# IST-DASLab/torch_cgx

Hardware: AMD Instinct MI355X
Metric: DDP samples/sec ResNet-50 4-bit (higher is better)
Workload: dtype bf16; 1 GPU; model=resnet50, global_batch=256, input=3x224x224, parallelism=dp1, backend=cgx, bits=4, bucket_size=1024, compression_active=False

## Files before the change

### csrc/bindings.cc

```cpp
#include <torch/extension.h>

#include <ATen/hip/impl/HIPStreamMasqueradingAsCUDA.h>
#include <torch/csrc/utils/pybind.h>

#include <ATen/hip/impl/HIPGuardImplMasqueradingAsCUDA.h>

#include <cstring>
#include <functional>
#include <thread>
#include <tuple>

#include "backend.h"
#include "bn_plan.h"
#include "collectives.h"
#include "reducer.h"

namespace cgx {
namespace {

void run_rank_threads(int ws, int dev,
                      const std::function<void(int, hipStream_t)>& body,
                      const std::function<void()>& abort) {
  std::vector<hipStream_t> qs(ws, nullptr);
  for (auto& s : qs)
    CGX_HIP_CHECK(hipStreamCreateWithFlags(&s, hipStreamNonBlocking));
  std::vector<std::exception_ptr> errs(ws);
  {
    py::gil_scoped_release nogil;
    std::vector<std::thread> th;
    for (int r = 0; r < ws; r++) {
      th.emplace_back([&, r] {
        try {
          c10::hip::HIPGuardMasqueradingAsCUDA g(dev);
          body(r, qs[r]);
        } catch (...) {
          errs[r] = std::current_exception();
          abort();
        }
      });
    }
    for (auto& t : th) t.join();
  }
  (void)hipDeviceSynchronize();
  for (auto s : qs)
    if (s) (void)hipStreamDestroy(s);
  for (int r = 0; r < ws; r++)
    if (errs[r]) std::rethrow_exception(errs[r]);
}

struct LoopbackWorld {
  std::vector<std::unique_ptr<LoopbackHub>> hubs;
  std::vector<std::unique_ptr<LoopbackTransport>> trs;
  std::vector<Reducer> ranks;

  LoopbackWorld(int ws, int local_size) {
    ranks.resize(ws);
    LoopbackHub* world = hub(ws);
    for (int r = 0; r < ws; r++) ranks[r].flat.emplace(r, ws, tr(world, r));
    if (local_size == 0) return;
    const int nodes = ws / local_size;
    LoopbackHub* cross = hub(nodes);
    for (int nd = 0; nd < nodes; nd++) {
      LoopbackHub* intra = hub(local_size);
      for (int lr = 0; lr < local_size; lr++) {
        Reducer& red = ranks[nd * local_size + lr];
        red.intra.emplace(lr, local_size, tr(intra, lr));
        red.leader = lr == 0;
        if (red.leader)
          red.cross.emplace(nd, nodes, tr(cross, nd), true);
      }
    }
  }
  void abort() {
    for (auto& h : hubs) h->abort();
  }

 private:
  LoopbackHub* hub(int world) {
    hubs.push_back(std::make_unique<LoopbackHub>(world));
    return hubs.back().get();
  }
  Transport* tr(LoopbackHub* h, int rank) {
    trs.push_back(std::make_unique<LoopbackTransport>(h, rank));
    return trs.back().get();
  }
};

void run_loopback(
    const std::vector<at::Tensor>& tensors, int local_size,
    const std::function<hipStream_t(Reducer&, hipStream_t, int)>& body) {
  const int ws = (int)tensors.size();
  TORCH_CHECK(ws >= 2, "loopback: need >= 2 per-rank tensors");
  TORCH_CHECK(local_size == 0 || (ws % local_size == 0 && ws / local_size >= 2),
              "loopback: hierarchical world must be n_nodes*local_size with "
              ">= 2 nodes");
  for (const auto& t : tensors) {
    TORCH_CHECK(t.is_cuda() && t.is_contiguous(),
                "loopback: CUDA contiguous tensors required");
    TORCH_CHECK(t.device() == tensors[0].device() &&
                    t.numel() == tensors[0].numel() &&
                    t.scalar_type() == tensors[0].scalar_type(),
                "loopback: tensors must match in device/numel/dtype");
  }
  const int dev = tensors[0].device().index();
  c10::hip::HIPGuardMasqueradingAsCUDA guard(dev);
  LoopbackWorld world(ws, local_size);
  run_rank_threads(
      ws, dev,
      [&](int r, hipStream_t qs) {
        hipStream_t fin = body(world.ranks[r], qs, r);
        CGX_HIP_CHECK(hipStreamSynchronize(fin));
        CGX_HIP_CHECK(hipStreamSynchronize(qs));
        world.ranks[r].for_each_stream(
            [](hipStream_t s) { CGX_HIP_CHECK(hipStreamSynchronize(s)); });
      },
      [&] { world.abort(); });
}

struct Resolved {
  explicit Resolved(int64_t numel)
      : matched(Registry::get().next(numel, nullptr, &info)) {}
  Registry::BucketInfo info;
  bool matched;
};

void py_loopback_allreduce(std::vector<at::Tensor> buckets) {
  const Resolved reg(buckets.empty() ? 0 : buckets[0].numel());
  run_loopback(buckets, 0,
               [&](Reducer& red, hipStream_t qs, int r) {
                 return red.allreduce(buckets[r], qs, &reg.info, reg.matched);
               });
}

void py_loopback_allreduce_multi(
    std::vector<std::vector<at::Tensor>> steps) {
  TORCH_CHECK(!steps.empty(), "loopback_allreduce_multi: no steps");
  const int ws = (int)steps[0].size();
  const int64_t numel = steps[0][0].numel();
  for (auto& st : steps) {
    TORCH_CHECK((int)st.size() == ws && st[0].numel() == numel,
                "loopback_allreduce_multi: ragged steps");
  }
  const Resolved reg(numel);
  run_loopback(steps[0], 0,
               [&](Reducer& red, hipStream_t qs, int r) {
                 hipStream_t fin = qs;
                 for (auto& st : steps)
                   fin = red.allreduce(st[r], qs, &reg.info, reg.matched);
                 return fin;
               });
}

void py_loopback_broadcast(std::vector<at::Tensor> tensors, int64_t root) {
  run_loopback(tensors, 0,
               [&](Reducer& red, hipStream_t qs, int r) {
                 return red.flat->engine->broadcast(tensors[r], (int)root,
                                                    red.flat->tr, qs);
               });
}

void py_loopback_hierarchical(std::vector<at::Tensor> buckets,
                              int64_t local_size) {
  TORCH_CHECK(local_size >= 1, "loopback_hierarchical: local_size >= 1");
  const Resolved reg(buckets.empty() ? 0 : buckets[0].numel());
  run_loopback(buckets, (int)local_size,
               [&](Reducer& red, hipStream_t qs, int r) {
                 return red.allreduce(buckets[r], qs, &reg.info, reg.matched);
               });
}

void py_loopback_collective(
    const std::string& name, std::vector<std::vector<at::Tensor>> inputs,
    std::vector<std::vector<at::Tensor>> outputs, int64_t root,
    std::vector<std::vector<int64_t>> in_splits,
    std::vector<std::vector<int64_t>> out_splits) {
  const int ws = (int)inputs.size();
  TORCH_CHECK(ws >= 1 && (int)outputs.size() == ws && root >= 0 && root < ws,
              "loopback_collective: one input and one output list per rank "
              "and a root among them");
  TORCH_CHECK((in_splits.empty() || (int)in_splits.size() == ws) &&
                  (out_splits.empty() || (int)out_splits.size() == ws),
              "loopback_collective: splits are per rank, or empty");
  in_splits.resize(ws);
  out_splits.resize(ws);
  std::function<size_t(int)> n_in, n_out;
  std::function<void(Transport*, int, hipStream_t)> call;
  const auto one = [](int) { return (size_t)1; };
  const auto all = [ws](int) { return (size_t)ws; };
  const auto at_root = [ws, root](int r) { return r == root ? (size_t)ws : 0; };
  if (name == "allgather") {
    n_in = one; n_out = all;
    call = [&](Transport* tr, int r, hipStream_t s) {
      coll::allgather(tr, r, ws, inputs[r][0], outputs[r], s);
    };
  } else if (name == "gather") {
    n_in = one; n_out = at_root;
    call = [&](Transport* tr, int r, hipStream_t s) {
      coll::gather(tr, r, ws, (int)root, inputs[r][0], outputs[r], s);
    };
  } else if (name == "scatter") {
    n_in = at_root; n_out = one;
    call = [&](Transport* tr, int r, hipStream_t s) {
      coll::scatter(tr, r, ws, (int)root, inputs[r], outputs[r][0], s);
    };
  } else if (name == "alltoall") {
    n_in = all; n_out = all;
    call = [&](Transport* tr, int r, hipStream_t s) {
      coll::alltoall(tr, r, ws, inputs[r], outputs[r], s);
    };
  } else if (name == "alltoall_base") {
    n_in = one; n_out = one;
    call = [&](Transport* tr, int r, hipStream_t s) {
      coll::alltoall_base(tr, r, ws, inputs[r][0], outputs[r][0], in_splits[r],
                          out_splits[r], s);
    };
  } else {
    TORCH_CHECK(false, "loopback_collective: unknown collective '", name, "'");
  }
  c10::optional<at::Device> device;
  for (int r = 0; r < ws; r++) {
    TORCH_CHECK(inputs[r].size() == n_in(r) && outputs[r].size() == n_out(r),
                "loopback_collective: rank ", r, " of ", name, " takes ",
                n_in(r), " input and ", n_out(r), " output tensors");
    for (const auto* ts : {&inputs[r], &outputs[r]})
      for (const at::Tensor& t : *ts) {
        TORCH_CHECK(t.is_cuda() && t.is_contiguous(),
                    "loopback_collective: CUDA contiguous tensors required");
        if (!device) device = t.device();
        TORCH_CHECK(t.device() == *device,
                    "loopback_collective: tensors must share one device");
      }
  }
  const int dev = device->index();
  c10::hip::HIPGuardMasqueradingAsCUDA guard(dev);
  CGX_HIP_CHECK(hipStreamSynchronize(
      c10::hip::getCurrentHIPStreamMasqueradingAsCUDA(dev).stream()));
  LoopbackHub hub(ws);
  std::vector<LoopbackTransport> trs;
  for (int r = 0; r < ws; r++) trs.emplace_back(&hub, r);
  run_rank_threads(
      ws, dev,
      [&](int r, hipStream_t s) {
        call(&trs[r], r, s);
        CGX_HIP_CHECK(hipStreamSynchronize(s));
      },
      [&] { hub.abort(); });
}

template <typename Desc>
at::Tensor upload(const std::vector<Desc>& descs,
                  const std::vector<int64_t>& cum, at::Device device) {
  const size_t desc_bytes = sizeof(Desc) * descs.size();
  const size_t cum_bytes = sizeof(int64_t) * cum.size();
  std::vector<char> host(desc_bytes + cum_bytes);
  std::memcpy(host.data(), descs.data(), desc_bytes);
  std::memcpy(host.data() + desc_bytes, cum.data(), cum_bytes);
  return at::from_blob(host.data(), {(int64_t)host.size()},
                       at::TensorOptions().dtype(at::kByte))
      .to(device);
}

void dequantize_slice(const at::Tensor& comp, at::Tensor& out, int64_t bits,
                      int64_t bucket_size, bool skip_incomplete,
                      int64_t src_stride, int nsrc, bool add) {
  const DType dt = dtype_of(out);
  auto stream =
      c10::hip::getCurrentHIPStreamMasqueradingAsCUDA(out.device().index());
  const std::vector<DequantSlice> slices{
      DequantSlice{comp.data_ptr<uint8_t>(), out.data_ptr(), out.numel(),
                   (int)bits, (int)bucket_size, skip_incomplete}};
  for (const DequantGroup& g :
       route_dequantize(slices, dt, src_stride, nsrc, add)) {
    auto dev = upload(g.descs, {}, out.device());
    launch(g, static_cast<const DequantDesc*>(dev.data_ptr()), dt,
           stream.stream());
  }
}

at::Tensor py_quantize(at::Tensor x, int64_t bits, int64_t bucket_size,
                       bool stochastic, int64_t seed, bool skip_incomplete,
                       c10::optional<at::Tensor> feedback) {
  TORCH_CHECK(x.is_cuda() && x.is_contiguous(), "quantize: CUDA contiguous");
  TORCH_CHECK(bits >= 1 && bits <= 8, "quantize: bits in [1,8]");
  TORCH_CHECK(bucket_size >= 1, "quantize: bucket_size >= 1");
  void* fbp = nullptr;
  if (feedback.has_value()) {
    TORCH_CHECK(feedback->is_cuda() && feedback->is_contiguous() &&
                    feedback->numel() == x.numel() &&
                    feedback->scalar_type() == x.scalar_type(),
                "quantize: feedback must match x");
    TORCH_CHECK(bucket_size % 8 == 0,
                "quantize: error feedback requires bucket_size % 8 == 0");
    fbp = feedback->data_ptr();
  }
  const DType dt = dtype_of(x);
  const int64_t n = x.numel();
  const int64_t bytes =
      buffer_size(n, dt, (int)bits, (int)bucket_size, skip_incomplete);
  auto out = at::zeros({std::max<int64_t>(bytes, 1)},
                       at::TensorOptions().dtype(at::kByte).device(x.device()));
  auto stream =
      c10::hip::getCurrentHIPStreamMasqueradingAsCUDA(x.device().index());
  for (const QuantGroup& g : route_quantize({QuantSlice{
           x.data_ptr(), out.data_ptr<uint8_t>(), fbp, n, (int)bits,
           (int)bucket_size, skip_incomplete}})) {
    auto dev = upload(g.descs, g.cum, x.device());
    const char* devp = static_cast<const char*>(dev.data_ptr());
    launch(g, reinterpret_cast<const QuantDesc*>(devp),
           reinterpret_cast<const int64_t*>(devp +
                                            sizeof(QuantDesc) * g.descs.size()),
           dt, (uint64_t)seed, stochastic, stream.stream());
  }
  return out;
}

void py_dequantize(at::Tensor comp, at::Tensor out, int64_t bits,
                   int64_t bucket_size, bool add, bool skip_incomplete) {
  TORCH_CHECK(comp.is_cuda() && out.is_cuda() && out.is_contiguous());
  dequantize_slice(comp, out, bits, bucket_size, skip_incomplete,
                   0, 1, add);
}

void py_dequantize_multi(at::Tensor comp, at::Tensor out, int64_t bits,
                         int64_t bucket_size, bool add) {
  TORCH_CHECK(comp.is_cuda() && comp.dim() == 2 && comp.is_contiguous());
  TORCH_CHECK(out.is_cuda() && out.is_contiguous());
  dequantize_slice(comp, out, bits, bucket_size, false,
                   comp.stride(0), (int)comp.size(0), add);
}

int64_t py_buffer_size(int64_t n, at::ScalarType st, int64_t bits,
                       int64_t bucket_size, bool skip_incomplete) {
  return buffer_size(n, dtype_of(st), (int)bits, (int)bucket_size,
                     skip_incomplete);
}

py::list py_route_quantize(
    const std::vector<std::tuple<uint64_t, uint64_t, uint64_t, int64_t, int,
                                 int, bool>>& slices) {
  std::vector<QuantSlice> qs;
  for (const auto& [in, out, fb, n, bits, bucket, skip] : slices)
    qs.push_back(QuantSlice{reinterpret_cast<const void*>(in),
                            reinterpret_cast<uint8_t*>(out),
                            reinterpret_cast<void*>(fb), n, bits, bucket,
                            skip});
  py::list groups;
  for (const QuantGroup& g : route_quantize(qs)) {
    py::list descs;
    for (const QuantDesc& d : g.descs)
      descs.append(py::make_tuple(reinterpret_cast<uint64_t>(d.in),
                                  reinterpret_cast<uint64_t>(d.out),
                                  reinterpret_cast<uint64_t>(d.fb), d.n,
                                  d.bucket, d.flags));
    groups.append(py::make_tuple(g.bits, g.kind, descs, g.cum, g.any_residual,
                                 g.max_gpl));
  }
  return groups;
}

py::list py_route_dequantize(
    const std::vector<std::tuple<uint64_t, uint64_t, int64_t, int, int,
                                 bool>>& slices,
    at::ScalarType st, int64_t src_stride, int nsrc, bool add) {
  std::vector<DequantSlice> ds;
  for (const auto& [in, out, n, bits, bucket, skip] : slices)
    ds.push_back(DequantSlice{reinterpret_cast<const uint8_t*>(in),
                              reinterpret_cast<void*>(out), n, bits, bucket,
                              skip});
  py::list groups;
  for (const DequantGroup& g :
       route_dequantize(ds, dtype_of(st), src_stride, nsrc, add)) {
    py::list descs;
    for (const DequantDesc& d : g.descs)
      descs.append(py::make_tuple(reinterpret_cast<uint64_t>(d.in),
                                  reinterpret_cast<uint64_t>(d.out), d.n,
                                  d.src_stride, d.bucket, d.nsrc, d.add,
                                  d.flags));
    groups.append(py::make_tuple(g.bits, g.kind, descs, g.total_groups,
                                 g.any_residual));
  }
  return groups;
}

std::pair<std::vector<int64_t>, std::vector<int64_t>> py_partition(
    int64_t num_elements, int64_t world_size,
    std::vector<int64_t> layer_numels, int64_t esize) {
  std::vector<int64_t> offs, szs;
  partition(num_elements, (int)world_size, layer_numels, (int)esize, &offs,
            &szs);
  return {offs, szs};
}

using PyView = std::tuple<uint64_t, int64_t, int, int>;
std::vector<LayerView> to_views(const std::vector<PyView>& views) {
  std::vector<LayerView> out;
  for (const auto& [off, numel, bits, bucket] : views)
    out.push_back(LayerView{reinterpret_cast<char*>(off), numel, bits, bucket});
  return out;
}

py::tuple py_plan_bucket(const std::vector<int64_t>& layer_numels,
                         const std::vector<std::pair<int, int>>& layer_cfgs,
                         at::ScalarType st, int64_t fusion_bytes,
                         int64_t min_elems, double fake_ratio, bool dummy) {
  TORCH_CHECK(layer_numels.size() == layer_cfgs.size(),
              "plan_bucket: one (bits, bucket_size) per layer");
  const int es = elem_size(dtype_of(st));
  EngineConfig cfg;
  cfg.fusion_bytes = fusion_bytes;
  cfg.min_elems = min_elems;
  cfg.fake_ratio = fake_ratio;
  cfg.dummy = dummy;
  std::vector<LayerView> views;
  int64_t off = 0;
  for (size_t i = 0; i < layer_numels.size(); i++) {
    views.push_back(LayerView{reinterpret_cast<char*>(off * es),
                              layer_numels[i], layer_cfgs[i].first,
                              layer_cfgs[i].second});
    off += layer_numels[i];
  }
  const BucketPlan bp = plan_bucket(views, cfg, es);
  py::list uncomp, chunks;
  for (const auto& [ptr, cnt] : bp.uncomp)
    uncomp.append(py::make_tuple(reinterpret_cast<uint64_t>(ptr), cnt));
  for (const auto& chunk : bp.chunks) {
    py::list vs;
    for (const LayerView& v : chunk)
      vs.append(py::make_tuple(reinterpret_cast<uint64_t>(v.data), v.numel,
                               v.bits, v.bucket_size));
    chunks.append(vs);
  }
  return py::make_tuple(uncomp, chunks);
}

py::tuple py_plan_chunk(const std::vector<PyView>& views, at::ScalarType st,
                        int ws, bool skip_incomplete) {
  TORCH_CHECK(ws >= 1, "plan_chunk: ws >= 1");
  const ChunkPlan pl =
      plan_chunk(to_views(views), dtype_of(st), ws, skip_incomplete);
  py::list rs;
  for (const auto& slices : pl.rs) {
    py::list r;
    for (const Slice& s : slices)
      r.append(py::make_tuple(reinterpret_cast<uint64_t>(s.data), s.n, s.bits,
                              s.bucket, s.comp_off, s.skip_incomplete,
                              s.fb_off));
    rs.append(r);
  }
  return py::make_tuple(pl.offs, pl.szs, pl.comp, rs);
}


bool bn_tensor_ok(const at::Tensor& t) {
  return t.is_cuda() && t.scalar_type() == at::kBFloat16 && t.dim() == 4 &&
         t.numel() > 0 && t.is_contiguous(at::MemoryFormat::ChannelsLast) &&
         reinterpret_cast<uintptr_t>(t.data_ptr()) % 16 == 0;
}

BnPlan bn_plan_of(const at::Tensor& t) {
  return bn_plan(t.numel() / t.size(1), t.size(1));
}

bool py_bn_eligible(const at::Tensor& x) {
  return bn_tensor_ok(x) && bn_plan_of(x).eligible;
}

float* bn_channel_vec(const at::Tensor& t, int64_t c, const char* what) {
  TORCH_CHECK(t.is_cuda() && t.scalar_type() == at::kFloat &&
                  t.is_contiguous() && t.numel() == c,
              "bn_act: ", what, " must be a contiguous fp32 CUDA vector of ",
              c, " elements");
  return t.data_ptr<float>();
}

at::Tensor bn_workspace(const BnPlan& p, const at::Tensor& like) {
  return at::empty({2 * p.partial_floats + p.grid},
                   like.options().dtype(at::kFloat));
}

std::tuple<at::Tensor, at::Tensor, at::Tensor, c10::optional<at::Tensor>>
py_bn_act_forward(const at::Tensor& x, const c10::optional<at::Tensor>& identity,
                  const at::Tensor& weight, const at::Tensor& bias,
                  at::Tensor running_mean, at::Tensor running_var,
                  double momentum, double eps, bool relu) {
  TORCH_CHECK(py_bn_eligible(x), "bn_act_forward: input is not eligible");
  const BnPlan p = bn_plan_of(x);
  const int64_t c = p.channels;
  if (identity.has_value())
    TORCH_CHECK(bn_tensor_ok(*identity) && identity->sizes() == x.sizes() &&
                    identity->device() == x.device(),
                "bn_act_forward: identity must match the input");
  c10::hip::HIPGuardMasqueradingAsCUDA guard(x.device().index());
  auto out = at::empty(x.sizes(), x.options(), at::MemoryFormat::ChannelsLast);
  auto stats = x.options().dtype(at::kFloat);
  auto mean = at::empty({c}, stats), invstd = at::empty({c}, stats);
  c10::optional<at::Tensor> mask;
  if (relu) mask = at::empty({x.numel() / 8}, x.options().dtype(at::kByte));
  auto part = bn_workspace(p, x);
  BnForwardArgs a;
  a.x = x.data_ptr();
  a.identity = identity.has_value() ? identity->data_ptr() : nullptr;
  a.weight = bn_channel_vec(weight, c, "weight");
  a.bias = bn_channel_vec(bias, c, "bias");
  a.running_mean = bn_channel_vec(running_mean, c, "running_mean");
  a.running_var = bn_channel_vec(running_var, c, "running_var");
  a.momentum = (float)momentum;
  a.eps = (float)eps;
  a.relu = relu;
  a.out = out.data_ptr();
  a.mean = mean.data_ptr<float>();
  a.invstd = invstd.data_ptr<float>();
  a.mask = relu ? mask->data_ptr<uint8_t>() : nullptr;
  a.part = part.data_ptr<float>();
  launch_bn_forward(
      p, a, c10::hip::getCurrentHIPStreamMasqueradingAsCUDA(
                x.device().index()).stream());
  return {out, mean, invstd, mask};
}

std::tuple<at::Tensor, at::Tensor, at::Tensor, c10::optional<at::Tensor>>
py_bn_act_backward(at::Tensor dy, const at::Tensor& x, const at::Tensor& mean,
                   const at::Tensor& invstd, const at::Tensor& weight,
                   const c10::optional<at::Tensor>& mask, bool has_identity) {
  TORCH_CHECK(py_bn_eligible(x), "bn_act_backward: input is not eligible");
  const BnPlan p = bn_plan_of(x);
  const int64_t c = p.channels;
  TORCH_CHECK(dy.is_cuda() && dy.device() == x.device() &&
                  dy.scalar_type() == at::kBFloat16 && dy.sizes() == x.sizes(),
              "bn_act_backward: dy must match the input");
  c10::hip::HIPGuardMasqueradingAsCUDA guard(x.device().index());
  if (!bn_tensor_ok(dy)) dy = dy.contiguous(at::MemoryFormat::ChannelsLast);
  if (!bn_tensor_ok(dy)) dy = dy.clone(at::MemoryFormat::ChannelsLast);
  if (mask.has_value())
    TORCH_CHECK(mask->is_cuda() && mask->scalar_type() == at::kByte &&
                    mask->is_contiguous() && mask->numel() == x.numel() / 8,
                "bn_act_backward: mask must hold one bit per element");
  auto dx = at::empty(x.sizes(), x.options(), at::MemoryFormat::ChannelsLast);
  auto stats = x.options().dtype(at::kFloat);
  auto dgamma = at::empty({c}, stats), dbeta = at::empty({c}, stats);
  c10::optional<at::Tensor> didentity;
  if (has_identity)
    didentity = mask.has_value()
                    ? at::empty(x.sizes(), x.options(),
                                at::MemoryFormat::ChannelsLast)
                    : dy;
  auto part = bn_workspace(p, x);
  BnBackwardArgs a;
  a.dy = dy.data_ptr();
  a.x = x.data_ptr();
  a.mean = bn_channel_vec(mean, c, "mean");
  a.invstd = bn_channel_vec(invstd, c, "invstd");
  a.weight = bn_channel_vec(weight, c, "weight");
  a.mask = mask.has_value() ? mask->data_ptr<uint8_t>() : nullptr;
  a.dx = dx.data_ptr();
  a.didentity =
      has_identity && mask.has_value() ? didentity->data_ptr() : nullptr;
  a.dgamma = dgamma.data_ptr<float>();
  a.dbeta = dbeta.data_ptr<float>();
  a.part = part.data_ptr<float>();
  launch_bn_backward(
      p, a, c10::hip::getCurrentHIPStreamMasqueradingAsCUDA(
                x.device().index()).stream());
  return {dx, dgamma, dbeta, didentity};
}

hipStream_t bn_stream(const at::Tensor& x) {
  return c10::hip::getCurrentHIPStreamMasqueradingAsCUDA(x.device().index())
      .stream();
}

at::Tensor bn_dense_dy(at::Tensor dy) {
  if (!bn_tensor_ok(dy)) dy = dy.contiguous(at::MemoryFormat::ChannelsLast);
  if (!bn_tensor_ok(dy)) dy = dy.clone(at::MemoryFormat::ChannelsLast);
  return dy;
}

std::tuple<at::Tensor, at::Tensor, at::Tensor, at::Tensor, at::Tensor,
           c10::optional<at::Tensor>>
py_bn_act2_forward(const at::Tensor& x3, const at::Tensor& xd,
                   const at::Tensor& weight3, const at::Tensor& bias3,
                   at::Tensor running_mean3, at::Tensor running_var3,
                   double momentum3, double eps3, const at::Tensor& weightd,
                   const at::Tensor& biasd, at::Tensor running_meand,
                   at::Tensor running_vard, double momentumd, double epsd,
                   bool relu) {
  TORCH_CHECK(py_bn_eligible(x3), "bn_act2_forward: input is not eligible");
  TORCH_CHECK(bn_tensor_ok(xd) && xd.sizes() == x3.sizes() &&
                  xd.device() == x3.device(),
              "bn_act2_forward: both inputs must have the same shape");
  const BnPlan p = bn_plan_of(x3);
  const int64_t c = p.channels;
  c10::hip::HIPGuardMasqueradingAsCUDA guard(x3.device().index());
  auto out = at::empty(x3.sizes(), x3.options(), at::MemoryFormat::ChannelsLast);
  auto stats = x3.options().dtype(at::kFloat);
  auto mean3 = at::empty({c}, stats), invstd3 = at::empty({c}, stats);
  auto meand = at::empty({c}, stats), invstdd = at::empty({c}, stats);
  c10::optional<at::Tensor> mask;
  if (relu) mask = at::empty({x3.numel() / 8}, x3.options().dtype(at::kByte));
  auto part = at::empty({2 * (2 * p.partial_floats + p.grid)}, stats);
  BnJoinArgs j{};
  j.a.x = x3.data_ptr();
  j.a.weight = bn_channel_vec(weight3, c, "weight");
  j.a.bias = bn_channel_vec(bias3, c, "bias");
  j.a.running_mean = bn_channel_vec(running_mean3, c, "running_mean");
  j.a.running_var = bn_channel_vec(running_var3, c, "running_var");
  j.a.momentum = (float)momentum3;
  j.a.eps = (float)eps3;
  j.a.mean = mean3.data_ptr<float>();
  j.a.invstd = invstd3.data_ptr<float>();
  j.b.x = xd.data_ptr();
  j.b.weight = bn_channel_vec(weightd, c, "identity weight");
  j.b.bias = bn_channel_vec(biasd, c, "identity bias");
  j.b.running_mean = bn_channel_vec(running_meand, c, "identity running_mean");
  j.b.running_var = bn_channel_vec(running_vard, c, "identity running_var");
  j.b.momentum = (float)momentumd;
  j.b.eps = (float)epsd;
  j.b.mean = meand.data_ptr<float>();
  j.b.invstd = invstdd.data_ptr<float>();
  j.relu = relu;
  j.out = out.data_ptr();
  j.mask = relu ? mask->data_ptr<uint8_t>() : nullptr;
  j.part = part.data_ptr<float>();
  launch_bn_join_forward(p, j, bn_stream(x3));
  return {out, mean3, invstd3, meand, invstdd, mask};
}

std::tuple<at::Tensor, at::Tensor, at::Tensor, at::Tensor, at::Tensor,
           at::Tensor>
py_bn_act2_backward(at::Tensor dy, const at::Tensor& x3, const at::Tensor& xd,
                    const at::Tensor& mean3, const at::Tensor& invstd3,
                    const at::Tensor& weight3, const at::Tensor& meand,
                    const at::Tensor& invstdd, const at::Tensor& weightd,
                    const c10::optional<at::Tensor>& mask) {
  TORCH_CHECK(py_bn_eligible(x3), "bn_act2_backward: input is not eligible");
  TORCH_CHECK(bn_tensor_ok(xd) && xd.sizes() == x3.sizes() &&
                  xd.device() == x3.device(),
              "bn_act2_backward: both inputs must have the same shape");
  const BnPlan p = bn_plan_of(x3);
  const int64_t c = p.channels;
  TORCH_CHECK(dy.is_cuda() && dy.device() == x3.device() &&
                  dy.scalar_type() == at::kBFloat16 && dy.sizes() == x3.sizes(),
              "bn_act2_backward: dy must match the input");
  c10::hip::HIPGuardMasqueradingAsCUDA guard(x3.device().index());
  dy = bn_dense_dy(dy);
  if (mask.has_value())
    TORCH_CHECK(mask->is_cuda() && mask->scalar_type() == at::kByte &&
                    mask->is_contiguous() && mask->numel() == x3.numel() / 8,
                "bn_act2_backward: mask must hold one bit per element");
  auto dx3 = at::empty(x3.sizes(), x3.options(), at::MemoryFormat::ChannelsLast);
  auto dxd = at::empty(x3.sizes(), x3.options(), at::MemoryFormat::ChannelsLast);
  auto stats = x3.options().dtype(at::kFloat);
  auto dgamma3 = at::empty({c}, stats), dbeta3 = at::empty({c}, stats);
  auto dgammad = at::empty({c}, stats), dbetad = at::empty({c}, stats);
  auto part = at::empty({3 * p.partial_floats}, stats);
  BnJoinArgs j{};
  j.a.x = x3.data_ptr();
  j.a.mean = bn_channel_vec(mean3, c, "mean");
  j.a.invstd = bn_channel_vec(invstd3, c, "invstd");
  j.a.weight = bn_channel_vec(weight3, c, "weight");
  j.a.dx = dx3.data_ptr();
  j.a.dgamma = dgamma3.data_ptr<float>();
  j.a.dbeta = dbeta3.data_ptr<float>();
  j.b.x = xd.data_ptr();
  j.b.mean = bn_channel_vec(meand, c, "identity mean");
  j.b.invstd = bn_channel_vec(invstdd, c, "identity invstd");
  j.b.weight = bn_channel_vec(weightd, c, "identity weight");
  j.b.dx = dxd.data_ptr();
  j.b.dgamma = dgammad.data_ptr<float>();
  j.b.dbeta = dbetad.data_ptr<float>();
  j.dy = dy.data_ptr();
  j.mask = mask.has_value() ? mask->data_ptr<uint8_t>() : nullptr;
  j.part = part.data_ptr<float>();
  launch_bn_join_backward(p, j, bn_stream(x3));
  return {dx3, dxd, dgamma3, dbeta3, dgammad, dbetad};
}

BnPoolPlan bn_pool_plan_of(const at::Tensor& x) {
  return bn_pool_plan(x.size(0), x.size(2), x.size(3), x.size(1));
}

std::tuple<at::Tensor, at::Tensor, at::Tensor, at::Tensor>
py_bn_act_pool_forward(const at::Tensor& x, const at::Tensor& weight,
                       const at::Tensor& bias, at::Tensor running_mean,
                       at::Tensor running_var, double momentum, double eps) {
  TORCH_CHECK(py_bn_eligible(x), "bn_act_pool_forward: input is not eligible");
  const BnPlan p = bn_plan_of(x);
  const BnPoolPlan g = bn_pool_plan_of(x);
  const int64_t c = p.channels;
  c10::hip::HIPGuardMasqueradingAsCUDA guard(x.device().index());
  auto out = at::empty({x.size(0), c, g.oh, g.ow}, x.options(),
                       at::MemoryFormat::ChannelsLast);
  auto arg = at::empty({x.size(0), c, g.oh, g.ow},
                       x.options().dtype(at::kByte),
                       at::MemoryFormat::ChannelsLast);
  auto stats = x.options().dtype(at::kFloat);
  auto mean = at::empty({c}, stats), invstd = at::empty({c}, stats);
  auto part = bn_workspace(p, x);
  BnPoolArgs a{};
  a.x = x.data_ptr();
  a.weight = bn_channel_vec(weight, c, "weight");
  a.bias = bn_channel_vec(bias, c, "bias");
  a.running_mean = bn_channel_vec(running_mean, c, "running_mean");
  a.running_var = bn_channel_vec(running_var, c, "running_var");
  a.momentum = (float)momentum;
  a.eps = (float)eps;
  a.mean = mean.data_ptr<float>();
  a.invstd = invstd.data_ptr<float>();
  a.out = out.data_ptr();
  a.arg = arg.data_ptr<uint8_t>();
  a.part = part.data_ptr<float>();
  launch_bn_pool_forward(p, g, a, bn_stream(x));
  return {out, mean, invstd, arg};
}

std::tuple<at::Tensor, at::Tensor, at::Tensor>
py_bn_act_pool_backward(at::Tensor dy, const at::Tensor& x,
                        const at::Tensor& mean, const at::Tensor& invstd,
                        const at::Tensor& weight, const at::Tensor& arg) {
  TORCH_CHECK(py_bn_eligible(x), "bn_act_pool_backward: input is not eligible");
  const BnPlan p = bn_plan_of(x);
  const BnPoolPlan g = bn_pool_plan_of(x);
  const int64_t c = p.channels;
  const std::vector<int64_t> pooled = {x.size(0), c, g.oh, g.ow};
  TORCH_CHECK(dy.is_cuda() && dy.device() == x.device() &&
                  dy.scalar_type() == at::kBFloat16 && dy.sizes() == at::IntArrayRef(pooled),
              "bn_act_pool_backward: dy must have the pooled shape");
  TORCH_CHECK(arg.is_cuda() && arg.device() == x.device() &&
                  arg.scalar_type() == at::kByte && arg.sizes() == at::IntArrayRef(pooled) &&
                  arg.is_contiguous(at::MemoryFormat::ChannelsLast) &&
                  reinterpret_cast<uintptr_t>(arg.data_ptr()) % 8 == 0,
              "bn_act_pool_backward: arg must be the forward's");
  c10::hip::HIPGuardMasqueradingAsCUDA guard(x.device().index());
  dy = bn_dense_dy(dy);
  auto dx = at::empty(x.sizes(), x.options(), at::MemoryFormat::ChannelsLast);
  auto stats = x.options().dtype(at::kFloat);
  auto dgamma = at::empty({c}, stats), dbeta = at::empty({c}, stats);
  auto part = bn_workspace(p, x);
  BnPoolArgs a{};
  a.x = x.data_ptr();
  a.mean = bn_channel_vec(mean, c, "mean");
  a.invstd = bn_channel_vec(invstd, c, "invstd");
  a.weight = bn_channel_vec(weight, c, "weight");
  a.arg = arg.data_ptr<uint8_t>();
  a.dy = dy.data_ptr();
  a.dx = dx.data_ptr();
  a.dgamma = dgamma.data_ptr<float>();
  a.dbeta = dbeta.data_ptr<float>();
  a.part = part.data_ptr<float>();
  launch_bn_pool_backward(p, g, a, bn_stream(x));
  return {dx, dgamma, dbeta};
}

std::tuple<at::Tensor, at::Tensor> py_bn_pool_geometry(int64_t h, int64_t w) {
  TORCH_CHECK(h >= 1 && w >= 1 && h * w <= kBnMaxRows, "bn_pool_geometry: bad");
  const BnPoolPlan g = bn_pool_plan(1, h, w, 8);
  auto opt = at::TensorOptions().dtype(at::kLong);
  auto windows = at::full({(int64_t)g.oh * g.ow, 9}, -1, opt);
  auto covers = at::full({h * w, 4, 2}, -1, opt);
  int64_t* wi = windows.data_ptr<int64_t>();
  int64_t* co = covers.data_ptr<int64_t>();
  for (int oh = 0; oh < g.oh; oh++)
    for (int ow = 0; ow < g.ow; ow++)
      for (int k = 0; k < 9; k++) {
        const int ih = pool_in(oh, k / 3), iw = pool_in(ow, k % 3);
        if (ih >= 0 && ih < g.h && iw >= 0 && iw < g.w)
          wi[((int64_t)oh * g.ow + ow) * 9 + k] = (int64_t)ih * g.w + iw;
      }
  for (int ih = 0; ih < g.h; ih++)
    for (int iw = 0; iw < g.w; iw++) {
      int n = 0;
      for (int oh = pool_cover_lo(ih); oh <= pool_cover_hi(ih, g.oh); oh++)
        for (int ow = pool_cover_lo(iw); ow <= pool_cover_hi(iw, g.ow); ow++) {
          int64_t* e = co + (((int64_t)ih * g.w + iw) * 4 + n++) * 2;
          e[0] = (int64_t)oh * g.ow + ow;
          e[1] = pool_k(ih, oh) * 3 + pool_k(iw, ow);
        }
    }
  return {windows, covers};
}

py::dict py_bn_plan(int64_t rows, int64_t channels) {
  const BnPlan p = bn_plan(rows, channels);
  py::dict d;
  d["eligible"] = p.eligible;
  d["threads"] = kBnThreads;
  d["cgs"] = p.cgs;
  d["tile_cgs"] = p.tc;
  d["ctiles"] = p.ctiles;
  d["rows_per_iter"] = p.rln;
  d["splits"] = p.splits;
  d["grid"] = p.grid;
  d["rows_per_thread"] = p.rows_per_thread;
  d["partial_floats"] = p.partial_floats;
  return d;
}

at::Tensor py_bn_sweep_indices(int64_t rows, int64_t channels) {
  const BnPlan p = bn_plan(rows, channels);
  TORCH_CHECK(p.eligible, "bn_sweep_indices: shape is not eligible");
  auto out = at::full({(int64_t)p.grid * kBnThreads, p.rows_per_thread + 1},
                      -1, at::TensorOptions().dtype(at::kLong));
  int64_t* o = out.data_ptr<int64_t>();
  const int64_t width = p.rows_per_thread + 1;
  for (int wg = 0; wg < p.grid; wg++)
    for (int tid = 0; tid < kBnThreads; tid++) {
      const BnSweep sw = bn_sweep(p, wg, tid);
      int64_t k = 0;
      for (int64_t r = sw.row; r < p.rows; r += sw.stride, k++) {
        TORCH_CHECK(k < width, "bn_sweep_indices: run longer than planned");
        o[((int64_t)wg * kBnThreads + tid) * width + k] = bn_vec(p, r, sw.cg);
      }
    }
  return out;
}

std::vector<int64_t> py_bn_partial_offsets(int64_t rows, int64_t channels,
                                           int wg) {
  const BnPlan p = bn_plan(rows, channels);
  TORCH_CHECK(p.eligible && wg >= 0 && wg < p.grid, "bn_partial_offsets: bad");
  std::vector<int64_t> offs;
  for (int tid = 0; tid < p.tc; tid++) {
    const BnSweep sw = bn_sweep(p, wg, tid);
    const int64_t o = bn_partial_offset(p, wg, sw.cg);
    for (int j = 0; j < 8; j++) offs.push_back(o + j);
  }
  return offs;
}

void py_register_layer(int64_t bucket_idx, int64_t layer_idx, int64_t numel,
                       int64_t bits, int64_t bucket_size) {
  Registry::get().register_layer((int)bucket_idx, (int)layer_idx, numel,
                                 (int)bits, (int)bucket_size);
}

void py_set_bits(int64_t bucket_idx, int64_t layer_idx, int64_t bits) {
  Registry::get().set_bits((int)bucket_idx, (int)layer_idx, (int)bits);
}

void py_set_bucket(int64_t bucket_idx, int64_t layer_idx,
                   int64_t bucket_size) {
  Registry::get().set_bucket_size((int)bucket_idx, (int)layer_idx,
                                  (int)bucket_size);
}

}
}

PYBIND11_MODULE(TORCH_EXTENSION_NAME, m) {
  py::class_<cgx::ProcessGroupCGX,
             c10::intrusive_ptr<cgx::ProcessGroupCGX>, c10d::Backend>(
      m, "ProcessGroupCGX")
      .def(py::init<c10::intrusive_ptr<c10d::Store>, int, int,
                    c10::intrusive_ptr<c10d::Backend>>(),
           py::arg("store"), py::arg("rank"), py::arg("size"),
           py::arg("cpu_delegate") = nullptr);

  m.def("register_layer", &cgx::py_register_layer, py::arg("bucket_idx"),
        py::arg("layer_idx"), py::arg("layer_numel"), py::arg("bits"),
        py::arg("bucket_size"));
  m.def("set_quantization_bits", &cgx::py_set_bits);
  m.def("set_quantization_bucket_size", &cgx::py_set_bucket);
  m.def("clear_registry", [] { cgx::Registry::get().clear(); });
  m.def("registry_match",
        [](int64_t numel, int64_t key) {
          cgx::Registry::BucketInfo info;
          const bool ok = cgx::Registry::get().next(
              numel, reinterpret_cast<const void*>(key), &info);
          return py::make_tuple(ok, ok ? info.idx : -1);
        },
        py::arg("numel"), py::arg("key") = 0);
  m.def("registry_snapshot", [] {
    py::list out;
    auto& reg = cgx::Registry::get();
    for (const auto& b : reg.snapshot()) {
      py::list numels, cfgs;
      for (auto n : b.numels) numels.append(n);
      for (const auto& c : b.cfgs)
        cfgs.append(py::make_tuple(c.bits, c.bucket_size));
      out.append(py::make_tuple(b.idx, numels, cfgs));
    }
    return out;
  });

  m.def("parse_engine_config", [] {
    auto c = cgx::EngineConfig::from_env();
    py::dict d;
    d["fusion_bytes"] = c.fusion_bytes;
    d["min_elems"] = c.min_elems;
    d["default_bits"] = c.default_bits;
    d["default_bucket"] = c.default_bucket;
    d["stochastic"] = c.stochastic;
    d["inner_ring"] = c.ring;
    d["cross_ring"] = c.cross_ring;
    d["debug_a2a"] = c.debug_a2a;
    d["fake_ratio"] = c.fake_ratio;
    d["skip_incomplete"] = c.skip_incomplete;
    d["dummy"] = c.dummy;
    d["intra_compress"] = c.intra_compress;
    d["intra_broadcast"] = c.intra_broadcast;
    d["error_feedback"] = c.error_feedback;
    return d;
  });
  m.def("env_flag", &cgx::env_flag, py::arg("name"),
        py::arg("default") = false,
        "Test seam: the textual boolean parser (only \"0\" is false).");
  m.def("env_int", &cgx::env_int, py::arg("name"), py::arg("default"),
        "Test seam: the numeric parser behind the `!= 0` booleans.");
  m.def("loopback_allreduce", &cgx::py_loopback_allreduce, py::arg("buckets"),
        "Run Reducer::allreduce (flat) at world_size=len(buckets) on one GPU "
        "via the loopback transport; buckets[r] is rank r's flat bucket "
        "tensor, reduced in place.");
  m.def("loopback_broadcast", &cgx::py_loopback_broadcast, py::arg("tensors"),
        py::arg("root") = 0,
        "Run the production Engine::broadcast at world_size=len(tensors) on "
        "one GPU via the loopback transport.");
  m.def("loopback_allreduce_multi", &cgx::py_loopback_allreduce_multi,
        py::arg("steps"),
        "Multiple allreduce steps on persistent engines (steps[s][r] = rank "
        "r's bucket at step s, reduced in place); error-feedback residuals "
        "carry across steps.");
  m.def("loopback_hierarchical", &cgx::py_loopback_hierarchical,
        py::arg("buckets"), py::arg("local_size"),
        "Run Reducer::allreduce, the backend's per-bucket call, for "
        "n_nodes*local_size ranks on one GPU via loopback transports: intra "
        "allreduce -> leader cross reduction -> intra broadcast, or the "
        "flat path under CGX_INTRA_BROADCAST=0.");
  m.def("loopback_collective", &cgx::py_loopback_collective, py::arg("name"),
        py::arg("inputs"), py::arg("outputs"), py::arg("root") = 0,
        py::arg("in_splits") = std::vector<std::vector<int64_t>>{},
        py::arg("out_splits") = std::vector<std::vector<int64_t>>{},
        "Run one of the backend's p2p collectives (allgather, gather, "
        "scatter, alltoall, alltoall_base) at world_size=len(inputs) on one "
        "GPU via the loopback transport; inputs[r] / outputs[r] are rank r's "
        "tensor lists, in_splits[r] / out_splits[r] its alltoall_base splits.");
  m.def("quantize", &cgx::py_quantize, py::arg("x"), py::arg("bits"),
        py::arg("bucket_size"), py::arg("stochastic") = false,
        py::arg("seed") = 0, py::arg("skip_incomplete") = false,
        py::arg("feedback") = py::none());
  m.def("dequantize", &cgx::py_dequantize, py::arg("comp"), py::arg("out"),
        py::arg("bits"), py::arg("bucket_size"), py::arg("add") = false,
        py::arg("skip_incomplete") = false);
  m.def("dequantize_multi", &cgx::py_dequantize_multi, py::arg("comp"),
        py::arg("out"), py::arg("bits"), py::arg("bucket_size"),
        py::arg("add") = false);
  m.def("compute_topology",
        [](const c10::intrusive_ptr<c10d::Store>& store, int rank, int size,
           const std::string& hostname) {
          auto t = cgx::compute_topology(store, rank, size, hostname);
          return std::make_tuple(t.node_id, t.local_rank, t.local_size,
                                 t.n_nodes, t.uniform);
        },
        "Exchange hostnames through the store -> (node_id, local_rank, "
        "local_size, n_nodes, uniform)");
  m.def("buffer_size", &cgx::py_buffer_size, py::arg("n"), py::arg("dtype"),
        py::arg("bits"), py::arg("bucket_size"),
        py::arg("skip_incomplete") = false);
  m.def("partition", &cgx::py_partition);
  m.def("plan_bucket", &cgx::py_plan_bucket, py::arg("layer_numels"),
        py::arg("layer_cfgs"), py::arg("dtype"), py::arg("fusion_bytes"),
        py::arg("min_elems"), py::arg("fake_ratio") = 1.0,
        py::arg("dummy") = false,
        "Test seam: the bucket plan for layers laid out back to back from "
        "byte offset 0 -> (uncomp [(byte_off, count)], chunks [[(byte_off, "
        "numel, bits, bucket)]]).");
  m.def("plan_chunk", &cgx::py_plan_chunk, py::arg("views"), py::arg("dtype"),
        py::arg("ws"), py::arg("skip_incomplete") = false,
        "Test seam: the rank plan of one chunk [(byte_off, numel, bits, "
        "bucket)] -> (offs, szs, comp, rs [[(byte_off, n, bits, bucket, "
        "comp_off, skip_incomplete, fb_off)]]).");
  m.def("route_quantize", &cgx::py_route_quantize, py::arg("slices"),
        "Test seam: the launch router's quantize plan for "
        "[(in, out, fb, n, bits, bucket, skip_incomplete)] (pointers as "
        "ints) -> [(bits, kind, descs, cum, any_residual, max_gpl)].");
  m.def("route_dequantize", &cgx::py_route_dequantize, py::arg("slices"),
        py::arg("dtype"), py::arg("src_stride") = 0, py::arg("nsrc") = 1,
        py::arg("add") = false,
        "Test seam: the launch router's dequantize plan for "
        "[(in, out, n, bits, bucket, skip_incomplete)] -> "
        "[(bits, kind, descs, total_groups, any_residual)].");
  m.def("bn_act_forward", &cgx::py_bn_act_forward, py::arg("x"),
        py::arg("identity"), py::arg("weight"), py::arg("bias"),
        py::arg("running_mean"), py::arg("running_var"), py::arg("momentum"),
        py::arg("eps"), py::arg("relu"),
        "Training-mode BatchNorm2d of a channels_last bf16 tensor, fused with "
        "an optional residual add and ReLU -> (out, mean, invstd, mask | "
        "None); updates the running statistics in place.");
  m.def("bn_act_backward", &cgx::py_bn_act_backward, py::arg("dy"),
        py::arg("x"), py::arg("mean"), py::arg("invstd"), py::arg("weight"),
        py::arg("mask"), py::arg("has_identity"),
        "Backward of bn_act_forward -> (dx, dgamma, dbeta, didentity | None).");
  m.def("bn_act2_forward", &cgx::py_bn_act2_forward,
        "relu(bn3(x3) + bn_d(xd)) with both BatchNorms in training mode: "
        "(x3, xd, weight3, bias3, running_mean3, running_var3, momentum3, "
        "eps3, weightd, biasd, running_meand, running_vard, momentumd, epsd, "
        "relu) -> (out, mean3, invstd3, meand, invstdd, mask | None).");
  m.def("bn_act2_backward", &cgx::py_bn_act2_backward,
        "Backward of bn_act2_forward: (dy, x3, xd, mean3, invstd3, weight3, "
        "meand, invstdd, weightd, mask) -> (dx3, dxd, dgamma3, dbeta3, "
        "dgammad, dbetad).");
  m.def("bn_act_pool_forward", &cgx::py_bn_act_pool_forward, py::arg("x"),
        py::arg("weight"), py::arg("bias"), py::arg("running_mean"),
        py::arg("running_var"), py::arg("momentum"), py::arg("eps"),
        "max_pool2d(relu(bn(x)), 3, 2, 1) in training mode -> (pooled, mean, "
        "invstd, arg); arg is one byte per pooled element.");
  m.def("bn_act_pool_backward", &cgx::py_bn_act_pool_backward, py::arg("dy"),
        py::arg("x"), py::arg("mean"), py::arg("invstd"), py::arg("weight"),
        py::arg("arg"),
        "Backward of bn_act_pool_forward -> (dx, dgamma, dbeta).");
  m.def("bn_pool_geometry", &cgx::py_bn_pool_geometry, py::arg("h"),
        py::arg("w"),
        "Test seam: (windows [oh*ow, 9], covers [h*w, 4, 2]) of the stem's "
        "3x3/2/1 pooling as the kernels index it.");
  m.def("bn_eligible", &cgx::py_bn_eligible, py::arg("x"),
        "True where the fused BatchNorm kernels take `x`: CUDA, bf16, dense "
        "channels_last, and a shape bn_plan calls eligible.");
  m.def("bn_plan", &cgx::py_bn_plan, py::arg("rows"), py::arg("channels"),
        "Test seam: the launch geometry of the fused BatchNorm kernels for a "
        "[rows, channels] activation.");
  m.def("bn_sweep_indices", &cgx::py_bn_sweep_indices, py::arg("rows"),
        py::arg("channels"),
        "Test seam: [grid*threads, rows_per_thread+1] int64, the 16-byte "
        "vector indices every thread visits (-1: none).");
  m.def("bn_partial_offsets", &cgx::py_bn_partial_offsets, py::arg("rows"),
        py::arg("channels"), py::arg("wg"),
        "Test seam: the partial-buffer floats workgroup `wg` writes.");
  m.attr("FLAG_SKIP_INCOMPLETE") = cgx::kFlagSkipIncomplete;
  m.attr("FLAG_TAIL_ONLY") = cgx::kFlagTailOnly;
  m.attr("KIND_FAST") = (int)cgx::kFast;
  m.attr("KIND_GENERIC") = (int)cgx::kGeneric;
  m.attr("KIND_TWO_PASS") = (int)cgx::kTwoPass;
  m.attr("KIND_SUB") = (int)cgx::kSub;
}
```

### csrc/bn_kernels.hip

```cpp
#include <hip/hip_runtime.h>

#include "bn_plan.h"
#include "check.h"

namespace cgx {
namespace {

constexpr int kT = kBnThreads;

__device__ inline void unpack8(const uint4& v, float (&f)[8]) {
  f[0] = __uint_as_float(v.x << 16);
  f[1] = __uint_as_float(v.x & 0xffff0000u);
  f[2] = __uint_as_float(v.y << 16);
  f[3] = __uint_as_float(v.y & 0xffff0000u);
  f[4] = __uint_as_float(v.z << 16);
  f[5] = __uint_as_float(v.z & 0xffff0000u);
  f[6] = __uint_as_float(v.w << 16);
  f[7] = __uint_as_float(v.w & 0xffff0000u);
}

__device__ inline unsigned bf16_bits(float f) {
  const unsigned u = __float_as_uint(f);
  if ((u & 0x7fffffffu) > 0x7f800000u) return (u >> 16) | 0x40u;
  return (u + 0x7fffu + ((u >> 16) & 1u)) >> 16;
}

__device__ inline uint4 pack8(const unsigned (&b)[8]) {
  return make_uint4(b[0] | (b[1] << 16), b[2] | (b[3] << 16),
                    b[4] | (b[5] << 16), b[6] | (b[7] << 16));
}

__device__ inline unsigned half_of(const uint4& v, int j) {
  const unsigned w = j < 2 ? v.x : j < 4 ? v.y : j < 6 ? v.z : v.w;
  return (j & 1) ? w >> 16 : w & 0xffffu;
}

template <int K>
__device__ inline void load_k(float (&dst)[K], const float* src) {
#pragma unroll
  for (int j = 0; j < K; j++) dst[j] = src[j];
}


template <int K>
struct Moments {
  float n = 0.f;
  float mean[K] = {};
  float m2[K] = {};

  __device__ void push(const float (&x)[K]) {
    n += 1.f;
    const float inv = __builtin_amdgcn_rcpf(n);
#pragma unroll
    for (int j = 0; j < K; j++) {
      const float d = x[j] - mean[j];
      mean[j] = fmaf(d, inv, mean[j]);
      m2[j] = fmaf(d, x[j] - mean[j], m2[j]);
    }
  }

  __device__ void merge(float nb, const float (&mb)[K], const float (&m2b)[K]) {
    const float nt = n + nb;
    const float fb = nt > 0.f ? nb / nt : 0.f;
    const float w = n * fb;
#pragma unroll
    for (int j = 0; j < K; j++) {
      const float d = mb[j] - mean[j];
      mean[j] = fmaf(d, fb, mean[j]);
      m2[j] = (m2[j] + m2b[j]) + (d * d) * w;
    }
    n = nt;
  }
};

template <int K>
__device__ inline void wg_merge(Moments<K>& m, float (*sh)[kT], int tid,
                                int lo) {
#pragma unroll
  for (int j = 0; j < K; j++) {
    sh[j][tid] = m.mean[j];
    sh[K + j][tid] = m.m2[j];
  }
  sh[2 * K][tid] = m.n;
  __syncthreads();
  for (int h = kT / 2; h >= lo; h >>= 1) {
    if (tid < h) {
      float mb[K], m2b[K];
#pragma unroll
      for (int j = 0; j < K; j++) {
        mb[j] = sh[j][tid + h];
        m2b[j] = sh[K + j][tid + h];
      }
      m.merge(sh[2 * K][tid + h], mb, m2b);
#pragma unroll
      for (int j = 0; j < K; j++) {
        sh[j][tid] = m.mean[j];
        sh[K + j][tid] = m.m2[j];
      }
      sh[2 * K][tid] = m.n;
    }
    __syncthreads();
  }
}

template <int K>
__device__ inline void wg_sum(float (&s)[K], float (*sh)[kT], int tid, int lo) {
#pragma unroll
  for (int j = 0; j < K; j++) sh[j][tid] = s[j];
  __syncthreads();
  for (int h = kT / 2; h >= lo; h >>= 1) {
    if (tid < h) {
#pragma unroll
      for (int j = 0; j < K; j++) {
        s[j] += sh[j][tid + h];
        sh[j][tid] = s[j];
      }
    }
    __syncthreads();
  }
}


__global__ __launch_bounds__(kT) void bn_stats(const uint4* __restrict__ x,
                                               float* __restrict__ pmean,
                                               float* __restrict__ pm2,
                                               float* __restrict__ pcnt,
                                               BnPlan p) {
  __shared__ float sh[17][kT];
  const int tid = threadIdx.x;
  const BnSweep sw = bn_sweep(p, blockIdx.x, tid);
  Moments<8> m;
  float f[8];
  int64_t r = sw.row;
  for (; r + 3 * sw.stride < p.rows; r += 4 * sw.stride) {
    const uint4 v0 = x[bn_vec(p, r, sw.cg)];
    const uint4 v1 = x[bn_vec(p, r + sw.stride, sw.cg)];
    const uint4 v2 = x[bn_vec(p, r + 2 * sw.stride, sw.cg)];
    const uint4 v3 = x[bn_vec(p, r + 3 * sw.stride, sw.cg)];
    unpack8(v0, f);
    m.push(f);
    unpack8(v1, f);
    m.push(f);
    unpack8(v2, f);
    m.push(f);
    unpack8(v3, f);
    m.push(f);
  }
  for (; r < p.rows; r += sw.stride) {
    unpack8(x[bn_vec(p, r, sw.cg)], f);
    m.push(f);
  }
  wg_merge<8>(m, sh, tid, p.tc);
  if (tid < p.tc) {
    const int64_t o = bn_partial_offset(p, blockIdx.x, sw.cg);
#pragma unroll
    for (int j = 0; j < 8; j++) {
      pmean[o + j] = m.mean[j];
      pm2[o + j] = m.m2[j];
    }
    if (tid == 0) pcnt[blockIdx.x] = m.n;
  }
}

constexpr int kFinLanes = kT / kBnFinChannels;

__global__ __launch_bounds__(kT) void bn_stats_finalize(
    const float* __restrict__ pmean, const float* __restrict__ pm2,
    const float* __restrict__ pcnt, float* __restrict__ mean,
    float* __restrict__ invstd, float* __restrict__ running_mean,
    float* __restrict__ running_var, float momentum, float eps, BnPlan p) {
  __shared__ float sh[3][kT];
  const int tid = threadIdx.x;
  const int c = blockIdx.x * kBnFinChannels + tid % kBnFinChannels;
  const int lane = tid / kBnFinChannels;
  Moments<1> m;
  if (c < p.channels) {
    const int ct = (c / 8) / p.tc;
    for (int s0 = lane; s0 < p.splits; s0 += 4 * kFinLanes) {
      float nb[4], mb[4][1], m2b[4][1];
#pragma unroll
      for (int u = 0; u < 4; u++) {
        const int s = s0 + u * kFinLanes;
        const bool live = s < p.splits;
        const int64_t o = (int64_t)s * p.channels + c;
        nb[u] = live ? pcnt[s * p.ctiles + ct] : 0.f;
        mb[u][0] = live ? pmean[o] : 0.f;
        m2b[u][0] = live ? pm2[o] : 0.f;
      }
#pragma unroll
      for (int u = 0; u < 4; u++) m.merge(nb[u], mb[u], m2b[u]);
    }
  }
  wg_merge<1>(m, sh, tid, kBnFinChannels);
  if (tid < kBnFinChannels && c < p.channels) {
    const float var = m.m2[0] / m.n;
    mean[c] = m.mean[0];
    invstd[c] = 1.f / sqrtf(var + eps);
    running_mean[c] =
        (1.f - momentum) * running_mean[c] + momentum * m.mean[0];
    running_var[c] =
        (1.f - momentum) * running_var[c] + momentum * (m.m2[0] / (m.n - 1.f));
  }
}

template <bool RELU, bool ADD>
__device__ inline void apply_one(const uint4& xv, const uint4& iv,
                                 const float (&mean)[8],
                                 const float (&invstd)[8],
                                 const float (&gamma)[8],
                                 const float (&beta)[8], uint4* out,
                                 uint8_t* mask, int64_t i) {
  float x[8], idn[8];
  unpack8(xv, x);
  if (ADD) unpack8(iv, idn);
  unsigned o[8], mbits = 0;
#pragma unroll
  for (int j = 0; j < 8; j++) {
    float y = ((x[j] - mean[j]) * invstd[j]) * gamma[j] + beta[j];
    unsigned b = bf16_bits(y);
    if (ADD) {
      y = __uint_as_float(b << 16) + idn[j];
      b = bf16_bits(y);
    }
    if (RELU) {
      const float z = __uint_as_float(b << 16);
      if (z <= 0.f) b = 0;
      else mbits |= 1u << j;
    }
    o[j] = b;
  }
  out[i] = pack8(o);
  if (RELU) mask[i] = (uint8_t)mbits;
}

template <bool RELU, bool ADD>
__global__ __launch_bounds__(kT) void bn_apply(
    const uint4* __restrict__ x, const uint4* __restrict__ identity,
    const float* __restrict__ mean_, const float* __restrict__ invstd_,
    const float* __restrict__ weight, const float* __restrict__ bias,
    uint4* __restrict__ out, uint8_t* __restrict__ mask, BnPlan p) {
  const BnSweep sw = bn_sweep(p, blockIdx.x, threadIdx.x);
  float mean[8], invstd[8], gamma[8], beta[8];
  load_k(mean, mean_ + sw.cg * 8);
  load_k(invstd, invstd_ + sw.cg * 8);
  load_k(gamma, weight + sw.cg * 8);
  load_k(beta, bias + sw.cg * 8);
  const uint4 none = make_uint4(0, 0, 0, 0);
  int64_t r = sw.row;
  for (; r + sw.stride < p.rows; r += 2 * sw.stride) {
    const int64_t i0 = bn_vec(p, r, sw.cg);
    const int64_t i1 = bn_vec(p, r + sw.stride, sw.cg);
    const uint4 x0 = x[i0], x1 = x[i1];
    const uint4 d0 = ADD ? identity[i0] : none, d1 = ADD ? identity[i1] : none;
    apply_one<RELU, ADD>(x0, d0, mean, invstd, gamma, beta, out, mask, i0);
    apply_one<RELU, ADD>(x1, d1, mean, invstd, gamma, beta, out, mask, i1);
  }
  if (r < p.rows) {
    const int64_t i0 = bn_vec(p, r, sw.cg);
    apply_one<RELU, ADD>(x[i0], ADD ? identity[i0] : none, mean, invstd, gamma,
                         beta, out, mask, i0);
  }
}


template <bool RELU>
__device__ inline void masked_dy(const uint4& dyv, unsigned mbits,
                                 float (&g)[8], unsigned (&gb)[8]) {
#pragma unroll
  for (int j = 0; j < 8; j++) {
    gb[j] = half_of(dyv, j);
    if (RELU && !((mbits >> j) & 1u)) gb[j] = 0;
    g[j] = __uint_as_float(gb[j] << 16);
  }
}

template <bool RELU>
__global__ __launch_bounds__(kT) void bn_bwd_reduce(
    const uint4* __restrict__ dy, const uint4* __restrict__ x,
    const uint8_t* __restrict__ mask, const float* __restrict__ mean_,
    const float* __restrict__ invstd_, float* __restrict__ psg,
    float* __restrict__ psgx, BnPlan p) {
  __shared__ float sh[16][kT];
  const int tid = threadIdx.x;
  const BnSweep sw = bn_sweep(p, blockIdx.x, tid);
  float mean[8], invstd[8];
  load_k(mean, mean_ + sw.cg * 8);
  load_k(invstd, invstd_ + sw.cg * 8);
  float s[16] = {};
  auto accumulate = [&](const uint4& dyv, const uint4& xv, unsigned mbits) {
    float g[8], xf[8];
    unsigned gb[8];
    masked_dy<RELU>(dyv, mbits, g, gb);
    unpack8(xv, xf);
#pragma unroll
    for (int j = 0; j < 8; j++) {
      const float xhat = (xf[j] - mean[j]) * invstd[j];
      s[j] += g[j];
      s[8 + j] = fmaf(g[j], xhat, s[8 + j]);
    }
  };
  int64_t r = sw.row;
  for (; r + sw.stride < p.rows; r += 2 * sw.stride) {
    const int64_t i0 = bn_vec(p, r, sw.cg);
    const int64_t i1 = bn_vec(p, r + sw.stride, sw.cg);
    const uint4 a0 = dy[i0], a1 = dy[i1];
    const uint4 b0 = x[i0], b1 = x[i1];
    const unsigned m0 = RELU ? mask[i0] : 0xffu, m1 = RELU ? mask[i1] : 0xffu;
    accumulate(a0, b0, m0);
    accumulate(a1, b1, m1);
  }
  if (r < p.rows) {
    const int64_t i0 = bn_vec(p, r, sw.cg);
    accumulate(dy[i0], x[i0], RELU ? mask[i0] : 0xffu);
  }
  wg_sum<16>(s, sh, tid, p.tc);
  if (tid < p.tc) {
    const int64_t o = bn_partial_offset(p, blockIdx.x, sw.cg);
#pragma unroll
    for (int j = 0; j < 8; j++) {
      psg[o + j] = s[j];
      psgx[o + j] = s[8 + j];
    }
  }
}

__global__ __launch_bounds__(kT) void bn_bwd_finalize(
    const float* __restrict__ psg, const float* __restrict__ psgx,
    float* __restrict__ dbeta, float* __restrict__ dgamma, BnPlan p) {
  __shared__ float sh[2][kT];
  const int tid = threadIdx.x;
  const int c = blockIdx.x * kBnFinChannels + tid % kBnFinChannels;
  const int lane = tid / kBnFinChannels;
  float s[2] = {0.f, 0.f};
  if (c < p.channels) {
    for (int s0 = lane; s0 < p.splits; s0 += 4 * kFinLanes) {
      float a[4], b[4];
#pragma unroll
      for (int u = 0; u < 4; u++) {
        const int sp = s0 + u * kFinLanes;
        const bool live = sp < p.splits;
        const int64_t o = (int64_t)sp * p.channels + c;
        a[u] = live ? psg[o] : 0.f;
        b[u] = live ? psgx[o] : 0.f;
      }
#pragma unroll
      for (int u = 0; u < 4; u++) {
        s[0] += a[u];
        s[1] += b[u];
      }
    }
  }
  wg_sum<2>(s, sh, tid, kBnFinChannels);
  if (tid < kBnFinChannels && c < p.channels) {
    dbeta[c] = s[0];
    dgamma[c] = s[1];
  }
}

template <bool RELU, bool ADD>
__global__ __launch_bounds__(kT) void bn_bwd_dx(
    const uint4* __restrict__ dy, const uint4* __restrict__ x,
    const uint8_t* __restrict__ mask, const float* __restrict__ mean_,
    const float* __restrict__ invstd_, const float* __restrict__ weight,
    const float* __restrict__ dbeta, const float* __restrict__ dgamma,
    uint4* __restrict__ dx, uint4* __restrict__ didentity, BnPlan p) {
  const BnSweep sw = bn_sweep(p, blockIdx.x, threadIdx.x);
  float mean[8], invstd[8], scale[8], mg[8], mgx[8];
  load_k(mean, mean_ + sw.cg * 8);
  load_k(invstd, invstd_ + sw.cg * 8);
  load_k(scale, weight + sw.cg * 8);
  load_k(mg, dbeta + sw.cg * 8);
  load_k(mgx, dgamma + sw.cg * 8);
  const float inv_r = 1.f / (float)p.rows;
#pragma unroll
  for (int j = 0; j < 8; j++) {
    scale[j] *= invstd[j];
    mg[j] *= inv_r;
    mgx[j] *= inv_r;
  }
  auto one = [&](const uint4& dyv, const uint4& xv, unsigned mbits, int64_t i) {
    float g[8], xf[8];
    unsigned gb[8], o[8];
    masked_dy<RELU>(dyv, mbits, g, gb);
    unpack8(xv, xf);
#pragma unroll
    for (int j = 0; j < 8; j++) {
      const float xhat = (xf[j] - mean[j]) * invstd[j];
      o[j] = bf16_bits(scale[j] * ((g[j] - mg[j]) - xhat * mgx[j]));
    }
    dx[i] = pack8(o);
    if (ADD) didentity[i] = pack8(gb);
  };
  int64_t r = sw.row;
  for (; r + sw.stride < p.rows; r += 2 * sw.stride) {
    const int64_t i0 = bn_vec(p, r, sw.cg);
    const int64_t i1 = bn_vec(p, r + sw.stride, sw.cg);
    const uint4 a0 = dy[i0], a1 = dy[i1];
    const uint4 b0 = x[i0], b1 = x[i1];
    const unsigned m0 = RELU ? mask[i0] : 0xffu, m1 = RELU ? mask[i1] : 0xffu;
    one(a0, b0, m0, i0);
    one(a1, b1, m1, i1);
  }
  if (r < p.rows) {
    const int64_t i0 = bn_vec(p, r, sw.cg);
    one(dy[i0], x[i0], RELU ? mask[i0] : 0xffu, i0);
  }
}


struct Affine {
  float mean[8], invstd[8], gamma[8], beta[8];
  __device__ void load(const float* mean_, const float* invstd_,
                       const float* weight, const float* bias, int cg) {
    load_k(mean, mean_ + cg * 8);
    load_k(invstd, invstd_ + cg * 8);
    load_k(gamma, weight + cg * 8);
    load_k(beta, bias + cg * 8);
  }
};

template <bool RELU>
__global__ __launch_bounds__(kT) void bn_apply_join(
    const uint4* __restrict__ x3, const uint4* __restrict__ xd,
    const float* __restrict__ mean3, const float* __restrict__ invstd3,
    const float* __restrict__ weight3, const float* __restrict__ bias3,
    const float* __restrict__ meand, const float* __restrict__ invstdd,
    const float* __restrict__ weightd, const float* __restrict__ biasd,
    uint4* __restrict__ out, uint8_t* __restrict__ mask, BnPlan p) {
  const BnSweep sw = bn_sweep(p, blockIdx.x, threadIdx.x);
  Affine a, b;
  a.load(mean3, invstd3, weight3, bias3, sw.cg);
  b.load(meand, invstdd, weightd, biasd, sw.cg);
  auto one = [&](const uint4& xv, const uint4& dv, int64_t i) {
    float d[8];
    unsigned idb[8];
    unpack8(dv, d);
#pragma unroll
    for (int j = 0; j < 8; j++)
      idb[j] = bf16_bits(((d[j] - b.mean[j]) * b.invstd[j]) * b.gamma[j] +
                         b.beta[j]);
    apply_one<RELU, true>(xv, pack8(idb), a.mean, a.invstd, a.gamma, a.beta,
                          out, mask, i);
  };
  int64_t r = sw.row;
  for (; r + sw.stride < p.rows; r += 2 * sw.stride) {
    const int64_t i0 = bn_vec(p, r, sw.cg);
    const int64_t i1 = bn_vec(p, r + sw.stride, sw.cg);
    const uint4 a0 = x3[i0], a1 = x3[i1];
    const uint4 d0 = xd[i0], d1 = xd[i1];
    one(a0, d0, i0);
    one(a1, d1, i1);
  }
  if (r < p.rows) {
    const int64_t i0 = bn_vec(p, r, sw.cg);
    one(x3[i0], xd[i0], i0);
  }
}

template <bool RELU>
__global__ __launch_bounds__(kT) void bn_bwd_reduce_join(
    const uint4* __restrict__ dy, const uint4* __restrict__ x3,
    const uint4* __restrict__ xd, const uint8_t* __restrict__ mask,
    const float* __restrict__ mean3_, const float* __restrict__ invstd3_,
    const float* __restrict__ meand_, const float* __restrict__ invstdd_,
    float* __restrict__ psg, float* __restrict__ psgx3,
    float* __restrict__ psgxd, BnPlan p) {
  __shared__ float sh[24][kT];
  const int tid = threadIdx.x;
  const BnSweep sw = bn_sweep(p, blockIdx.x, tid);
  float mean3[8], invstd3[8], meand[8], invstdd[8];
  load_k(mean3, mean3_ + sw.cg * 8);
  load_k(invstd3, invstd3_ + sw.cg * 8);
  load_k(meand, meand_ + sw.cg * 8);
  load_k(invstdd, invstdd_ + sw.cg * 8);
  float s[24] = {};
  auto accumulate = [&](const uint4& dyv, const uint4& av, const uint4& bv,
                        unsigned mbits) {
    float g[8], af[8], bf[8];
    unsigned gb[8];
    masked_dy<RELU>(dyv, mbits, g, gb);
    unpack8(av, af);
    unpack8(bv, bf);
#pragma unroll
    for (int j = 0; j < 8; j++) {
      const float xhat3 = (af[j] - mean3[j]) * invstd3[j];
      const float xhatd = (bf[j] - meand[j]) * invstdd[j];
      s[j] += g[j];
      s[8 + j] = fmaf(g[j], xhat3, s[8 + j]);
      s[16 + j] = fmaf(g[j], xhatd, s[16 + j]);
    }
  };
  int64_t r = sw.row;
  for (; r + sw.stride < p.rows; r += 2 * sw.stride) {
    const int64_t i0 = bn_vec(p, r, sw.cg);
    const int64_t i1 = bn_vec(p, r + sw.stride, sw.cg);
    const uint4 a0 = dy[i0], a1 = dy[i1];
    const uint4 b0 = x3[i0], b1 = x3[i1];
    const uint4 c0 = xd[i0], c1 = xd[i1];
    const unsigned m0 = RELU ? mask[i0] : 0xffu, m1 = RELU ? mask[i1] : 0xffu;
    accumulate(a0, b0, c0, m0);
    accumulate(a1, b1, c1, m1);
  }
  if (r < p.rows) {
    const int64_t i0 = bn_vec(p, r, sw.cg);
    accumulate(dy[i0], x3[i0], xd[i0], RELU ? mask[i0] : 0xffu);
  }
  wg_sum<24>(s, sh, tid, p.tc);
  if (tid < p.tc) {
    const int64_t o = bn_partial_offset(p, blockIdx.x, sw.cg);
#pragma unroll
    for (int j = 0; j < 8; j++) {
      psg[o + j] = s[j];
      psgx3[o + j] = s[8 + j];
      psgxd[o + j] = s[16 + j];
    }
  }
}

template <bool RELU>
__global__ __launch_bounds__(kT) void bn_bwd_dx_join(
    const uint4* __restrict__ dy, const uint4* __restrict__ x3,
    const uint4* __restrict__ xd, const uint8_t* __restrict__ mask,
    const float* __restrict__ mean3_, const float* __restrict__ invstd3_,
    const float* __restrict__ weight3, const float* __restrict__ dgamma3,
    const float* __restrict__ meand_, const float* __restrict__ invstdd_,
    const float* __restrict__ weightd, const float* __restrict__ dgammad,
    const float* __restrict__ dbeta, uint4* __restrict__ dx3,
    uint4* __restrict__ dxd, BnPlan p) {
  const BnSweep sw = bn_sweep(p, blockIdx.x, threadIdx.x);
  float mean3[8], invstd3[8], scale3[8], mgx3[8];
  float meand[8], invstdd[8], scaled[8], mgxd[8], mg[8];
  load_k(mean3, mean3_ + sw.cg * 8);
  load_k(invstd3, invstd3_ + sw.cg * 8);
  load_k(scale3, weight3 + sw.cg * 8);
  load_k(mgx3, dgamma3 + sw.cg * 8);
  load_k(meand, meand_ + sw.cg * 8);
  load_k(invstdd, invstdd_ + sw.cg * 8);
  load_k(scaled, weightd + sw.cg * 8);
  load_k(mgxd, dgammad + sw.cg * 8);
  load_k(mg, dbeta + sw.cg * 8);
  const float inv_r = 1.f / (float)p.rows;
#pragma unroll
  for (int j = 0; j < 8; j++) {
    scale3[j] *= invstd3[j];
    scaled[j] *= invstdd[j];
    mg[j] *= inv_r;
    mgx3[j] *= inv_r;
    mgxd[j] *= inv_r;
  }
  auto one = [&](const uint4& dyv, const uint4& av, const uint4& bv,
                 unsigned mbits, int64_t i) {
    float g[8], af[8], bf[8];
    unsigned gb[8], o3[8], od[8];
    masked_dy<RELU>(dyv, mbits, g, gb);
    unpack8(av, af);
    unpack8(bv, bf);
#pragma unroll
    for (int j = 0; j < 8; j++) {
      const float xhat3 = (af[j] - mean3[j]) * invstd3[j];
      const float xhatd = (bf[j] - meand[j]) * invstdd[j];
      o3[j] = bf16_bits(scale3[j] * ((g[j] - mg[j]) - xhat3 * mgx3[j]));
      od[j] = bf16_bits(scaled[j] * ((g[j] - mg[j]) - xhatd * mgxd[j]));
    }
    dx3[i] = pack8(o3);
    dxd[i] = pack8(od);
  };
  int64_t r = sw.row;
  for (; r + sw.stride < p.rows; r += 2 * sw.stride) {
    const int64_t i0 = bn_vec(p, r, sw.cg);
    const int64_t i1 = bn_vec(p, r + sw.stride, sw.cg);
    const uint4 a0 = dy[i0], a1 = dy[i1];
    const uint4 b0 = x3[i0], b1 = x3[i1];
    const uint4 c0 = xd[i0], c1 = xd[i1];
    const unsigned m0 = RELU ? mask[i0] : 0xffu, m1 = RELU ? mask[i1] : 0xffu;
    one(a0, b0, c0, m0, i0);
    one(a1, b1, c1, m1, i1);
  }
  if (r < p.rows) {
    const int64_t i0 = bn_vec(p, r, sw.cg);
    one(dy[i0], x3[i0], xd[i0], RELU ? mask[i0] : 0xffu, i0);
  }
}


__global__ __launch_bounds__(kT) void bn_apply_pool(
    const uint4* __restrict__ x, const float* __restrict__ mean_,
    const float* __restrict__ invstd_, const float* __restrict__ weight,
    const float* __restrict__ bias, uint4* __restrict__ out,
    uint2* __restrict__ arg, BnPoolPlan g) {
  const int64_t t = (int64_t)blockIdx.x * kT + threadIdx.x;
  if (t >= g.threads) return;
  const int cg = (int)(t % g.cgs);
  int pix = (int)(t / g.cgs);
  const int ow = pix % g.ow;
  pix /= g.ow;
  const int oh = pix % g.oh, n = pix / g.oh;
  float mean[8], invstd[8], gamma[8], beta[8];
  load_k(mean, mean_ + cg * 8);
  load_k(invstd, invstd_ + cg * 8);
  load_k(gamma, weight + cg * 8);
  load_k(beta, bias + cg * 8);
  uint4 v[9];
  bool live[9];
#pragma unroll
  for (int k = 0; k < 9; k++) {
    const int ih = pool_in(oh, k / 3), iw = pool_in(ow, k % 3);
    live[k] = ih >= 0 && ih < g.h && iw >= 0 && iw < g.w;
    v[k] = live[k] ? x[(((int64_t)n * g.h + ih) * g.w + iw) * g.cgs + cg]
                   : make_uint4(0, 0, 0, 0);
  }
  float best[8];
  unsigned bits[8], pos[8];
#pragma unroll
  for (int j = 0; j < 8; j++) {
    best[j] = -INFINITY;
    bits[j] = 0;
    pos[j] = kPoolNone;
  }
#pragma unroll
  for (int k = 0; k < 9; k++) {
    if (!live[k]) continue;
    float f[8];
    unpack8(v[k], f);
#pragma unroll
    for (int j = 0; j < 8; j++) {
      const float y = ((f[j] - mean[j]) * invstd[j]) * gamma[j] + beta[j];
      unsigned b = bf16_bits(y);
      float z = __uint_as_float(b << 16);
      if (z <= 0.f) {
        b = 0;
        z = 0.f;
      }
      if (z > best[j] || z != z) {
        best[j] = z;
        bits[j] = b;
        pos[j] = k;
      }
    }
  }
#pragma unroll
  for (int j = 0; j < 8; j++)
    if (best[j] <= 0.f) pos[j] = kPoolNone;
  out[t] = pack8(bits);
  arg[t] = make_uint2(pos[0] | (pos[1] << 8) | (pos[2] << 16) | (pos[3] << 24),
                      pos[4] | (pos[5] << 8) | (pos[6] << 16) | (pos[7] << 24));
}

__device__ inline void pooled_g(const uint4* __restrict__ dy,
                                const uint2* __restrict__ arg,
                                const BnPoolPlan& pl, int64_t row, int cg,
                                float (&g)[8]) {
  int pix = (int)row;
  const int iw = pix % pl.w;
  pix /= pl.w;
  const int ih = pix % pl.h, n = pix / pl.h;
  const int oh0 = pool_cover_lo(ih), oh1 = pool_cover_hi(ih, pl.oh);
  const int ow0 = pool_cover_lo(iw), ow1 = pool_cover_hi(iw, pl.ow);
  float acc[8] = {};
  for (int oh = oh0; oh <= oh1; oh++)
    for (int ow = ow0; ow <= ow1; ow++) {
      const int64_t i = (((int64_t)n * pl.oh + oh) * pl.ow + ow) * pl.cgs + cg;
      const unsigned k = pool_k(ih, oh) * 3 + pool_k(iw, ow);
      const uint4 dv = dy[i];
      const uint2 av = arg[i];
      float d[8];
      unpack8(dv, d);
#pragma unroll
      for (int j = 0; j < 8; j++) {
        const unsigned a = ((j < 4 ? av.x : av.y) >> (8 * (j & 3))) & 0xffu;
        if (a == k) acc[j] += d[j];
      }
    }
#pragma unroll
  for (int j = 0; j < 8; j++) g[j] = __uint_as_float(bf16_bits(acc[j]) << 16);
}

__global__ __launch_bounds__(kT) void bn_pool_bwd_reduce(
    const uint4* __restrict__ dy, const uint2* __restrict__ arg,
    const uint4* __restrict__ x, const float* __restrict__ mean_,
    const float* __restrict__ invstd_, float* __restrict__ psg,
    float* __restrict__ psgx, BnPlan p, BnPoolPlan pl) {
  __shared__ float sh[16][kT];
  const int tid = threadIdx.x;
  const BnSweep sw = bn_sweep(p, blockIdx.x, tid);
  float mean[8], invstd[8];
  load_k(mean, mean_ + sw.cg * 8);
  load_k(invstd, invstd_ + sw.cg * 8);
  float s[16] = {};
#pragma unroll 2
  for (int64_t r = sw.row; r < p.rows; r += sw.stride) {
    const uint4 xv = x[bn_vec(p, r, sw.cg)];
    float g[8], xf[8];
    pooled_g(dy, arg, pl, r, sw.cg, g);
    unpack8(xv, xf);
#pragma unroll
    for (int j = 0; j < 8; j++) {
      const float xhat = (xf[j] - mean[j]) * invstd[j];
      s[j] += g[j];
      s[8 + j] = fmaf(g[j], xhat, s[8 + j]);
    }
  }
  wg_sum<16>(s, sh, tid, p.tc);
  if (tid < p.tc) {
    const int64_t o = bn_partial_offset(p, blockIdx.x, sw.cg);
#pragma unroll
    for (int j = 0; j < 8; j++) {
      psg[o + j] = s[j];
      psgx[o + j] = s[8 + j];
    }
  }
}

__global__ __launch_bounds__(kT) void bn_pool_bwd_dx(
    const uint4* __restrict__ dy, const uint2* __restrict__ arg,
    const uint4* __restrict__ x, const float* __restrict__ mean_,
    const float* __restrict__ invstd_, const float* __restrict__ weight,
    const float* __restrict__ dbeta, const float* __restrict__ dgamma,
    uint4* __restrict__ dx, BnPlan p, BnPoolPlan pl) {
  const BnSweep sw = bn_sweep(p, blockIdx.x, threadIdx.x);
  float mean[8], invstd[8], scale[8], mg[8], mgx[8];
  load_k(mean, mean_ + sw.cg * 8);
  load_k(invstd, invstd_ + sw.cg * 8);
  load_k(scale, weight + sw.cg * 8);
  load_k(mg, dbeta + sw.cg * 8);
  load_k(mgx, dgamma + sw.cg * 8);
  const float inv_r = 1.f / (float)p.rows;
#pragma unroll
  for (int j = 0; j < 8; j++) {
    scale[j] *= invstd[j];
    mg[j] *= inv_r;
    mgx[j] *= inv_r;
  }
#pragma unroll 2
  for (int64_t r = sw.row; r < p.rows; r += sw.stride) {
    const int64_t i = bn_vec(p, r, sw.cg);
    const uint4 xv = x[i];
    float g[8], xf[8];
    unsigned o[8];
    pooled_g(dy, arg, pl, r, sw.cg, g);
    unpack8(xv, xf);
#pragma unroll
    for (int j = 0; j < 8; j++) {
      const float xhat = (xf[j] - mean[j]) * invstd[j];
      o[j] = bf16_bits(scale[j] * ((g[j] - mg[j]) - xhat * mgx[j]));
    }
    dx[i] = pack8(o);
  }
}

int fin_grid(const BnPlan& p) {
  return (p.channels + kBnFinChannels - 1) / kBnFinChannels;
}

void launch_bn_stats(const BnPlan& p, const void* x_, float* part, float* mean,
                     float* invstd, float* running_mean, float* running_var,
                     float momentum, float eps, hipStream_t stream) {
  float* pmean = part;
  float* pm2 = part + p.partial_floats;
  float* pcnt = part + 2 * p.partial_floats;
  const uint4* x = static_cast<const uint4*>(x_);
  hipLaunchKernelGGL(bn_stats, dim3(p.grid), dim3(kT), 0, stream, x, pmean,
                     pm2, pcnt, p);
  hipLaunchKernelGGL(bn_stats_finalize, dim3(fin_grid(p)), dim3(kT), 0, stream,
                     pmean, pm2, pcnt, mean, invstd, running_mean, running_var,
                     momentum, eps, p);
}

}

void launch_bn_forward(const BnPlan& p, const BnForwardArgs& a,
                       hipStream_t stream) {
  const uint4* x = static_cast<const uint4*>(a.x);
  const uint4* idn = static_cast<const uint4*>(a.identity);
  uint4* out = static_cast<uint4*>(a.out);
  const dim3 grid(p.grid), block(kT);
  launch_bn_stats(p, a.x, a.part, a.mean, a.invstd, a.running_mean,
                  a.running_var, a.momentum, a.eps, stream);
#define CGX_BN_APPLY(RELU, ADD)                                              \
  hipLaunchKernelGGL((bn_apply<RELU, ADD>), grid, block, 0, stream, x, idn,  \
                     a.mean, a.invstd, a.weight, a.bias, out, a.mask, p)
  if (a.relu && idn) CGX_BN_APPLY(true, true);
  else if (a.relu) CGX_BN_APPLY(true, false);
  else if (idn) CGX_BN_APPLY(false, true);
  else CGX_BN_APPLY(false, false);
#undef CGX_BN_APPLY
  CGX_HIP_CHECK(hipGetLastError());
}

void launch_bn_backward(const BnPlan& p, const BnBackwardArgs& a,
                        hipStream_t stream) {
  float* psg = a.part;
  float* psgx = a.part + p.partial_floats;
  const uint4* dy = static_cast<const uint4*>(a.dy);
  const uint4* x = static_cast<const uint4*>(a.x);
  uint4* dx = static_cast<uint4*>(a.dx);
  uint4* did = static_cast<uint4*>(a.didentity);
  const dim3 grid(p.grid), block(kT);
  if (a.mask)
    hipLaunchKernelGGL(bn_bwd_reduce<true>, grid, block, 0, stream, dy, x,
                       a.mask, a.mean, a.invstd, psg, psgx, p);
  else
    hipLaunchKernelGGL(bn_bwd_reduce<false>, grid, block, 0, stream, dy, x,
                       a.mask, a.mean, a.invstd, psg, psgx, p);
  hipLaunchKernelGGL(bn_bwd_finalize, dim3(fin_grid(p)), block, 0, stream, psg,
                     psgx, a.dbeta, a.dgamma, p);
#define CGX_BN_DX(RELU, ADD)                                                 \
  hipLaunchKernelGGL((bn_bwd_dx<RELU, ADD>), grid, block, 0, stream, dy, x,  \
                     a.mask, a.mean, a.invstd, a.weight, a.dbeta, a.dgamma,  \
                     dx, did, p)
  if (a.mask && did) CGX_BN_DX(true, true);
  else if (a.mask) CGX_BN_DX(true, false);
  else CGX_BN_DX(false, false);
#undef CGX_BN_DX
  CGX_HIP_CHECK(hipGetLastError());
}

void launch_bn_join_forward(const BnPlan& p, const BnJoinArgs& j,
                            hipStream_t stream) {
  const BnOperand &a = j.a, &b = j.b;
  float* part_b = j.part + 2 * p.partial_floats + p.grid;
  launch_bn_stats(p, a.x, j.part, a.mean, a.invstd, a.running_mean,
                  a.running_var, a.momentum, a.eps, stream);
  launch_bn_stats(p, b.x, part_b, b.mean, b.invstd, b.running_mean,
                  b.running_var, b.momentum, b.eps, stream);
  const uint4* x3 = static_cast<const uint4*>(a.x);
  const uint4* xd = static_cast<const uint4*>(b.x);
  uint4* out = static_cast<uint4*>(j.out);
  const dim3 grid(p.grid), block(kT);
  if (j.relu)
    hipLaunchKernelGGL(bn_apply_join<true>, grid, block, 0, stream, x3, xd,
                       a.mean, a.invstd, a.weight, a.bias, b.mean, b.invstd,
                       b.weight, b.bias, out, j.mask, p);
  else
    hipLaunchKernelGGL(bn_apply_join<false>, grid, block, 0, stream, x3, xd,
                       a.mean, a.invstd, a.weight, a.bias, b.mean, b.invstd,
                       b.weight, b.bias, out, j.mask, p);
  CGX_HIP_CHECK(hipGetLastError());
}

void launch_bn_join_backward(const BnPlan& p, const BnJoinArgs& j,
                             hipStream_t stream) {
  const BnOperand &a = j.a, &b = j.b;
  float* psg = j.part;
  float* psgx3 = j.part + p.partial_floats;
  float* psgxd = j.part + 2 * p.partial_floats;
  const uint4* dy = static_cast<const uint4*>(j.dy);
  const uint4* x3 = static_cast<const uint4*>(a.x);
  const uint4* xd = static_cast<const uint4*>(b.x);
  uint4* dx3 = static_cast<uint4*>(a.dx);
  uint4* dxd = static_cast<uint4*>(b.dx);
  const dim3 grid(p.grid), block(kT), fin(fin_grid(p));
  if (j.mask)
    hipLaunchKernelGGL(bn_bwd_reduce_join<true>, grid, block, 0, stream, dy, x3,
                       xd, j.mask, a.mean, a.invstd, b.mean, b.invstd, psg,
                       psgx3, psgxd, p);
  else
    hipLaunchKernelGGL(bn_bwd_reduce_join<false>, grid, block, 0, stream, dy,
                       x3, xd, j.mask, a.mean, a.invstd, b.mean, b.invstd, psg,
                       psgx3, psgxd, p);
  hipLaunchKernelGGL(bn_bwd_finalize, fin, block, 0, stream, psg, psgx3,
                     a.dbeta, a.dgamma, p);
  hipLaunchKernelGGL(bn_bwd_finalize, fin, block, 0, stream, psg, psgxd,
                     b.dbeta, b.dgamma, p);
  if (j.mask)
    hipLaunchKernelGGL(bn_bwd_dx_join<true>, grid, block, 0, stream, dy, x3, xd,
                       j.mask, a.mean, a.invstd, a.weight, a.dgamma, b.mean,
                       b.invstd, b.weight, b.dgamma, a.dbeta, dx3, dxd, p);
  else
    hipLaunchKernelGGL(bn_bwd_dx_join<false>, grid, block, 0, stream, dy, x3,
                       xd, j.mask, a.mean, a.invstd, a.weight, a.dgamma, b.mean,
                       b.invstd, b.weight, b.dgamma, a.dbeta, dx3, dxd, p);
  CGX_HIP_CHECK(hipGetLastError());
}

void launch_bn_pool_forward(const BnPlan& p, const BnPoolPlan& g,
                            const BnPoolArgs& a, hipStream_t stream) {
  launch_bn_stats(p, a.x, a.part, a.mean, a.invstd, a.running_mean,
                  a.running_var, a.momentum, a.eps, stream);
  hipLaunchKernelGGL(bn_apply_pool, dim3(g.grid), dim3(kT), 0, stream,
                     static_cast<const uint4*>(a.x), a.mean, a.invstd, a.weight,
                     a.bias, static_cast<uint4*>(a.out),
                     reinterpret_cast<uint2*>(a.arg), g);
  CGX_HIP_CHECK(hipGetLastError());
}

void launch_bn_pool_backward(const BnPlan& p, const BnPoolPlan& g,
                             const BnPoolArgs& a, hipStream_t stream) {
  float* psg = a.part;
  float* psgx = a.part + p.partial_floats;
  const uint4* dy = static_cast<const uint4*>(a.dy);
  const uint2* arg = reinterpret_cast<const uint2*>(a.arg);
  const uint4* x = static_cast<const uint4*>(a.x);
  const dim3 grid(p.grid), block(kT);
  hipLaunchKernelGGL(bn_pool_bwd_reduce, grid, block, 0, stream, dy, arg, x,
                     a.mean, a.invstd, psg, psgx, p, g);
  hipLaunchKernelGGL(bn_bwd_finalize, dim3(fin_grid(p)), block, 0, stream, psg,
                     psgx, a.dbeta, a.dgamma, p);
  hipLaunchKernelGGL(bn_pool_bwd_dx, grid, block, 0, stream, dy, arg, x, a.mean,
                     a.invstd, a.weight, a.dbeta, a.dgamma,
                     static_cast<uint4*>(a.dx), p, g);
  CGX_HIP_CHECK(hipGetLastError());
}

}
```

### csrc/bn_plan.h

```cpp
#pragma once

#include <hip/hip_runtime.h>

#include <cstdint>

namespace cgx {

constexpr int kBnThreads = 256;
constexpr int kBnTargetWgs = 1024;
constexpr int kBnMaxTileCgs = 32;
constexpr int kBnFinChannels = 4;

struct BnPlan {
  int64_t rows = 0;
  int channels = 0;
  bool eligible = false;
  int cgs = 0;
  int tc = 0;
  int ctiles = 0;
  int rln = 0;
  int splits = 0;
  int grid = 0;
  int rows_per_thread = 0;
  int64_t partial_floats = 0;
};

constexpr int64_t kBnMaxRows = int64_t(1) << 24;
BnPlan bn_plan(int64_t rows, int64_t channels);

struct BnSweep {
  int cg;
  int64_t row;
  int64_t stride;
};

__host__ __device__ inline BnSweep bn_sweep(const BnPlan& p, int wg, int tid) {
  const int ct = wg % p.ctiles, split = wg / p.ctiles;
  return BnSweep{ct * p.tc + tid % p.tc,
                 (int64_t)split * p.rln + tid / p.tc,
                 (int64_t)p.splits * p.rln};
}

__host__ __device__ inline int64_t bn_vec(const BnPlan& p, int64_t row,
                                          int cg) {
  return row * p.cgs + cg;
}

__host__ __device__ inline int64_t bn_partial_offset(const BnPlan& p, int wg,
                                                     int cg) {
  return (int64_t)(wg / p.ctiles) * p.channels + (int64_t)cg * 8;
}

struct BnForwardArgs {
  const void* x;
  const void* identity;
  const float* weight;
  const float* bias;
  float* running_mean;
  float* running_var;
  float momentum, eps;
  bool relu;
  void* out;
  float* mean;
  float* invstd;
  uint8_t* mask;
  float* part;
};
void launch_bn_forward(const BnPlan& p, const BnForwardArgs& a,
                       hipStream_t stream);

struct BnBackwardArgs {
  const void* dy;
  const void* x;
  const float* mean;
  const float* invstd;
  const float* weight;
  const uint8_t* mask;
  void* dx;
  void* didentity;
  float* dgamma;
  float* dbeta;
  float* part;
};
void launch_bn_backward(const BnPlan& p, const BnBackwardArgs& a,
                        hipStream_t stream);

struct BnOperand {
  const void* x;
  const float* weight;
  const float* bias;
  float* running_mean;
  float* running_var;
  float momentum, eps;
  float* mean;
  float* invstd;
  void* dx;
  float* dgamma;
  float* dbeta;
};
struct BnJoinArgs {
  BnOperand a, b;
  bool relu;
  void* out;
  const void* dy;
  uint8_t* mask;
  float* part;
};
void launch_bn_join_forward(const BnPlan& p, const BnJoinArgs& a,
                            hipStream_t stream);
void launch_bn_join_backward(const BnPlan& p, const BnJoinArgs& a,
                             hipStream_t stream);

constexpr int kPoolNone = 9;

struct BnPoolPlan {
  int n = 0, h = 0, w = 0;
  int oh = 0, ow = 0;
  int cgs = 0;
  int64_t threads = 0;
  int grid = 0;
};
BnPoolPlan bn_pool_plan(int64_t n, int64_t h, int64_t w, int64_t channels);

__host__ __device__ inline int pool_out(int in) { return (in - 1) / 2 + 1; }
__host__ __device__ inline int pool_in(int o, int k) { return 2 * o - 1 + k; }
__host__ __device__ inline int pool_cover_lo(int i) { return i / 2; }
__host__ __device__ inline int pool_cover_hi(int i, int out) {
  const int hi = (i + 1) / 2;
  return hi < out ? hi : out - 1;
}
__host__ __device__ inline int pool_k(int i, int o) { return i - (2 * o - 1); }

struct BnPoolArgs {
  const void* x;
  const float* weight;
  const float* bias;
  float* running_mean;
  float* running_var;
  float momentum, eps;
  float* mean;
  float* invstd;
  void* out;
  uint8_t* arg;
  const void* dy;
  void* dx;
  float* dgamma;
  float* dbeta;
  float* part;
};
void launch_bn_pool_forward(const BnPlan& p, const BnPoolPlan& g,
                            const BnPoolArgs& a, hipStream_t stream);
void launch_bn_pool_backward(const BnPlan& p, const BnPoolPlan& g,
                             const BnPoolArgs& a, hipStream_t stream);

}
```

### torch_cgx_amd/models/resnet.py

```python

from __future__ import annotations

import torch
import torch.nn as nn

from ..ops.fused_bn import bn_act, bn_act_pool


class Bottleneck(nn.Module):
    expansion = 4

    def __init__(self, inplanes: int, planes: int, stride: int = 1,
                 downsample: nn.Module = None):
        super().__init__()
        self.conv1 = nn.Conv2d(inplanes, planes, 1, bias=False)
        self.bn1 = nn.BatchNorm2d(planes)
        self.conv2 = nn.Conv2d(planes, planes, 3, stride=stride, padding=1,
                               bias=False)
        self.bn2 = nn.BatchNorm2d(planes)
        self.conv3 = nn.Conv2d(planes, planes * self.expansion, 1, bias=False)
        self.bn3 = nn.BatchNorm2d(planes * self.expansion)
        self.relu = nn.ReLU(inplace=True)
        self.downsample = downsample
        self.stride = stride

    def forward(self, x):
        identity = x
        out = bn_act(self.bn1, self.conv1(x))
        out = bn_act(self.bn2, self.conv2(out))
        out = self.conv3(out)
        if self.downsample is not None:
            conv, bn = self.downsample[0], self.downsample[1]
            return bn_act(self.bn3, out, conv(x), identity_bn=bn)
        return bn_act(self.bn3, out, identity)


class ResNet(nn.Module):
    def __init__(self, layers, num_classes: int = 1000):
        super().__init__()
        self.inplanes = 64
        self.conv1 = nn.Conv2d(3, 64, 7, stride=2, padding=3, bias=False)
        self.bn1 = nn.BatchNorm2d(64)
        self.relu = nn.ReLU(inplace=True)
        self.maxpool = nn.MaxPool2d(3, stride=2, padding=1)
        self.layer1 = self._make_layer(64, layers[0])
        self.layer2 = self._make_layer(128, layers[1], stride=2)
        self.layer3 = self._make_layer(256, layers[2], stride=2)
        self.layer4 = self._make_layer(512, layers[3], stride=2)
        self.avgpool = nn.AdaptiveAvgPool2d(1)
        self.fc = nn.Linear(512 * Bottleneck.expansion, num_classes)
        for m in self.modules():
            if isinstance(m, nn.Conv2d):
                nn.init.kaiming_normal_(m.weight, mode="fan_out",
                                        nonlinearity="relu")
            elif isinstance(m, nn.BatchNorm2d):
                nn.init.constant_(m.weight, 1)
                nn.init.constant_(m.bias, 0)

    def _make_layer(self, planes: int, blocks: int, stride: int = 1):
        downsample = None
        if stride != 1 or self.inplanes != planes * Bottleneck.expansion:
            downsample = nn.Sequential(
                nn.Conv2d(self.inplanes, planes * Bottleneck.expansion, 1,
                          stride=stride, bias=False),
                nn.BatchNorm2d(planes * Bottleneck.expansion),
            )
        layers = [Bottleneck(self.inplanes, planes, stride, downsample)]
        self.inplanes = planes * Bottleneck.expansion
        for _ in range(1, blocks):
            layers.append(Bottleneck(self.inplanes, planes))
        return nn.Sequential(*layers)

    def forward(self, x):
        x = bn_act_pool(self.bn1, self.conv1(x), self.maxpool)
        x = self.layer4(self.layer3(self.layer2(self.layer1(x))))
        x = self.avgpool(x).flatten(1)
        return self.fc(x)


def resnet50(num_classes: int = 1000) -> ResNet:
    return ResNet([3, 4, 6, 3], num_classes)


def resnet18(num_classes: int = 1000) -> nn.Module:

    class BasicBlock(nn.Module):
        def __init__(self, inp, planes, stride=1, down=None):
            super().__init__()
            self.c1 = nn.Conv2d(inp, planes, 3, stride, 1, bias=False)
            self.b1 = nn.BatchNorm2d(planes)
            self.c2 = nn.Conv2d(planes, planes, 3, 1, 1, bias=False)
            self.b2 = nn.BatchNorm2d(planes)
            self.down = down

        def forward(self, x):
            idt = x if self.down is None else self.down(x)
            out = torch.relu(self.b1(self.c1(x)))
            return torch.relu(self.b2(self.c2(out)) + idt)

    class R18(nn.Module):
        def __init__(self):
            super().__init__()
            self.stem = nn.Sequential(
                nn.Conv2d(3, 64, 7, 2, 3, bias=False), nn.BatchNorm2d(64),
                nn.ReLU(inplace=True), nn.MaxPool2d(3, 2, 1))
            chans = [64, 128, 256, 512]
            blocks = []
            inp = 64
            for i, c in enumerate(chans):
                stride = 1 if i == 0 else 2
                down = None
                if stride != 1 or inp != c:
                    down = nn.Sequential(nn.Conv2d(inp, c, 1, stride,
                                                   bias=False),
                                         nn.BatchNorm2d(c))
                blocks += [BasicBlock(inp, c, stride, down), ]
                inp = c
                blocks += [BasicBlock(c, c)]
            self.body = nn.Sequential(*blocks)
            self.head = nn.Linear(512, num_classes)

        def forward(self, x):
            x = self.body(self.stem(x))
            return self.head(torch.nn.functional.adaptive_avg_pool2d(
                x, 1).flatten(1))

    return R18()
```

### torch_cgx_amd/ops/fused_bn.py

```python

from __future__ import annotations

import os

import torch
import torch.nn.functional as F

from .. import _C


class _BnAct(torch.autograd.Function):
    @staticmethod
    def forward(ctx, x, identity, weight, bias, running_mean, running_var,
                momentum, eps, relu):
        out, mean, invstd, mask = _C.bn_act_forward(
            x, identity, weight, bias, running_mean, running_var, momentum,
            eps, relu)
        ctx.save_for_backward(x, mean, invstd, weight, mask)
        ctx.has_identity = identity is not None
        return out

    @staticmethod
    def backward(ctx, dy):
        x, mean, invstd, weight, mask = ctx.saved_tensors
        dx, dgamma, dbeta, didentity = _C.bn_act_backward(
            dy, x, mean, invstd, weight, mask, ctx.has_identity)
        return (dx, didentity, dgamma, dbeta, None, None, None, None, None)


class _BnActJoin(torch.autograd.Function):
    @staticmethod
    def forward(ctx, x, xd, weight, bias, running_mean, running_var, momentum,
                eps, weightd, biasd, running_meand, running_vard, momentumd,
                epsd, relu):
        out, mean, invstd, meand, invstdd, mask = _C.bn_act2_forward(
            x, xd, weight, bias, running_mean, running_var, momentum, eps,
            weightd, biasd, running_meand, running_vard, momentumd, epsd, relu)
        ctx.save_for_backward(x, xd, mean, invstd, weight, meand, invstdd,
                              weightd, mask)
        return out

    @staticmethod
    def backward(ctx, dy):
        (x, xd, mean, invstd, weight, meand, invstdd, weightd,
         mask) = ctx.saved_tensors
        dx, dxd, dgamma, dbeta, dgammad, dbetad = _C.bn_act2_backward(
            dy, x, xd, mean, invstd, weight, meand, invstdd, weightd, mask)
        return (dx, dxd, dgamma, dbeta, None, None, None, None, dgammad,
                dbetad, None, None, None, None, None)


class _BnActPool(torch.autograd.Function):
    @staticmethod
    def forward(ctx, x, weight, bias, running_mean, running_var, momentum,
                eps):
        out, mean, invstd, arg = _C.bn_act_pool_forward(
            x, weight, bias, running_mean, running_var, momentum, eps)
        ctx.save_for_backward(x, mean, invstd, weight, arg)
        return out

    @staticmethod
    def backward(ctx, dy):
        x, mean, invstd, weight, arg = ctx.saved_tensors
        dx, dgamma, dbeta = _C.bn_act_pool_backward(dy, x, mean, invstd,
                                                    weight, arg)
        return (dx, dgamma, dbeta, None, None, None, None)


def fused_bn_enabled() -> bool:
    return os.environ.get("CGX_FUSED_BN", "1") != "0"


def _native(bn, x, identity) -> bool:
    if not (bn.training and bn.track_running_stats
            and bn.momentum is not None and fused_bn_enabled()):
        return False
    if bn.weight is None or bn.bias is None:
        return False
    if not (x.is_cuda and _C.bn_eligible(x)):
        return False
    if identity is not None and not (
            identity.shape == x.shape and identity.device == x.device
            and _C.bn_eligible(identity)):
        return False
    return bn.weight.dtype == torch.float32


def _bn_args(bn):
    return (bn.weight, bn.bias, bn.running_mean, bn.running_var, bn.momentum,
            bn.eps)


def bn_act(bn: torch.nn.BatchNorm2d, x: torch.Tensor,
           identity: torch.Tensor = None, relu: bool = True,
           identity_bn: torch.nn.BatchNorm2d = None) -> torch.Tensor:
    if identity_bn is not None:
        if _native(bn, x, identity) and _native(identity_bn, identity, x):
            bn.num_batches_tracked.add_(1)
            identity_bn.num_batches_tracked.add_(1)
            return _BnActJoin.apply(x, identity, *_bn_args(bn),
                                    *_bn_args(identity_bn), relu)
        out = bn(x) + identity_bn(identity)
        return F.relu(out, inplace=True) if relu else out
    if _native(bn, x, identity):
        bn.num_batches_tracked.add_(1)
        return _BnAct.apply(x, identity, *_bn_args(bn), relu)
    out = bn(x)
    if identity is not None:
        out = out + identity
    if relu:
        out = F.relu(out, inplace=True)
    return out


def _pool_is_3x3_s2_p1(pool) -> bool:
    def pair(v):
        return tuple(v) if isinstance(v, (tuple, list)) else (v, v)

    return (type(pool) is torch.nn.MaxPool2d
            and pair(pool.kernel_size) == (3, 3) and pair(pool.stride) == (2, 2)
            and pair(pool.padding) == (1, 1) and pair(pool.dilation) == (1, 1)
            and not pool.ceil_mode and not pool.return_indices)


def bn_act_pool(bn: torch.nn.BatchNorm2d, x: torch.Tensor,
                pool: torch.nn.Module) -> torch.Tensor:
    if _pool_is_3x3_s2_p1(pool) and _native(bn, x, None):
        bn.num_batches_tracked.add_(1)
        return _BnActPool.apply(x, *_bn_args(bn))
    return pool(bn_act(bn, x))
```

Measured before the change: 7499 samples/s.

## Fuse BatchNorm statistics into a native 1x1 convolution kernel epilogue

Adds a custom MFMA-based 1x1 convolution kernel that writes per-channel BatchNorm partial moments (count, mean, M2) alongside its output. The fused BN forward then skips its own statistics pass over the conv output and only runs the finalize. The Bottleneck blocks route conv1, conv3 and the downsample conv through this path when the plan marks the shape native. This removes a full read of each 1x1 conv output, but replaces the vendor GEMM/conv with a hand-written kernel whose throughput may be lower.

```diff
diff --git a/csrc/bindings.cc b/csrc/bindings.cc
--- a/csrc/bindings.cc
+++ b/csrc/bindings.cc
@@ -13,6 +13,7 @@
 #include "backend.h"
 #include "bn_plan.h"
 #include "collectives.h"
+#include "conv1x1_plan.h"
 #include "reducer.h"
 
 namespace cgx {
@@ -473,6 +474,20 @@
   return t.data_ptr<float>();
 }
 
+BnPartials bn_external_partials(const at::Tensor& part, const at::Tensor& x) {
+  const int64_t c = x.size(1);
+  TORCH_CHECK(part.is_cuda() && part.device() == x.device() &&
+                  part.scalar_type() == at::kFloat && part.dim() == 2 &&
+                  part.is_contiguous() && part.size(0) >= 1 &&
+                  part.size(1) > 2 * c,
+              "bn_act: part must be the [splits, 2*C + ntiles] fp32 partials "
+              "of conv1x1_stats");
+  const int64_t ntiles = part.size(1) - 2 * c;
+  TORCH_CHECK(c % (8 * ntiles) == 0, "bn_act: part has a bad count column");
+  return conv1x1_partials(part.data_ptr<float>(), (int)c, (int)part.size(0),
+                          (int)ntiles);
+}
+
 at::Tensor bn_workspace(const BnPlan& p, const at::Tensor& like) {
   return at::empty({2 * p.partial_floats + p.grid},
                    like.options().dtype(at::kFloat));
@@ -482,7 +497,8 @@
 py_bn_act_forward(const at::Tensor& x, const c10::optional<at::Tensor>& identity,
                   const at::Tensor& weight, const at::Tensor& bias,
                   at::Tensor running_mean, at::Tensor running_var,
-                  double momentum, double eps, bool relu) {
+                  double momentum, double eps, bool relu,
+                  const c10::optional<at::Tensor>& stats_part) {
   TORCH_CHECK(py_bn_eligible(x), "bn_act_forward: input is not eligible");
   const BnPlan p = bn_plan_of(x);
   const int64_t c = p.channels;
@@ -512,6 +528,11 @@
   a.invstd = invstd.data_ptr<float>();
   a.mask = relu ? mask->data_ptr<uint8_t>() : nullptr;
   a.part = part.data_ptr<float>();
+  BnPartials ext;
+  if (stats_part.has_value()) {
+    ext = bn_external_partials(*stats_part, x);
+    a.stats = &ext;
+  }
   launch_bn_forward(
       p, a, c10::hip::getCurrentHIPStreamMasqueradingAsCUDA(
                 x.device().index()).stream());
@@ -583,7 +604,8 @@
                    double momentum3, double eps3, const at::Tensor& weightd,
                    const at::Tensor& biasd, at::Tensor running_meand,
                    at::Tensor running_vard, double momentumd, double epsd,
-                   bool relu) {
+                   bool relu, const c10::optional<at::Tensor>& stats_part3,
+                   const c10::optional<at::Tensor>& stats_partd) {
   TORCH_CHECK(py_bn_eligible(x3), "bn_act2_forward: input is not eligible");
   TORCH_CHECK(bn_tensor_ok(xd) && xd.sizes() == x3.sizes() &&
                   xd.device() == x3.device(),
@@ -621,6 +643,15 @@
   j.out = out.data_ptr();
   j.mask = relu ? mask->data_ptr<uint8_t>() : nullptr;
   j.part = part.data_ptr<float>();
+  BnPartials ext3, extd;
+  if (stats_part3.has_value()) {
+    ext3 = bn_external_partials(*stats_part3, x3);
+    j.a.stats = &ext3;
+  }
+  if (stats_partd.has_value()) {
+    extd = bn_external_partials(*stats_partd, xd);
+    j.b.stats = &extd;
+  }
   launch_bn_join_forward(p, j, bn_stream(x3));
   return {out, mean3, invstd3, meand, invstdd, mask};
 }
@@ -825,6 +856,86 @@
     for (int j = 0; j < 8; j++) offs.push_back(o + j);
   }
   return offs;
+}
+
+
+Conv1x1Plan conv1x1_plan_of(const at::Tensor& x, const at::Tensor& weight,
+                            int64_t max_workgroups) {
+  return conv1x1_plan(x.numel() / x.size(1), x.size(1), weight.size(0),
+                      (int)std::min<int64_t>(max_workgroups, 1 << 20));
+}
+
+bool py_conv1x1_eligible(const at::Tensor& x, const at::Tensor& weight) {
+  return bn_tensor_ok(x) && weight.is_cuda() &&
+         weight.device() == x.device() &&
+         weight.scalar_type() == at::kBFloat16 && weight.dim() == 4 &&
+         weight.size(1) == x.size(1) && weight.size(2) == 1 &&
+         weight.size(3) == 1 && weight.is_contiguous() &&
+         reinterpret_cast<uintptr_t>(weight.data_ptr()) % 16 == 0 &&
+         conv1x1_plan_of(x, weight, 0).eligible;
+}
+
+std::tuple<at::Tensor, at::Tensor> py_conv1x1_stats(const at::Tensor& x,
+                                                    const at::Tensor& weight,
+                                                    int64_t max_workgroups) {
+  TORCH_CHECK(max_workgroups >= 0, "conv1x1_stats: max_workgroups >= 0");
+  TORCH_CHECK(py_conv1x1_eligible(x, weight),
+              "conv1x1_stats: input or weight is not eligible");
+  const Conv1x1Plan p = conv1x1_plan_of(x, weight, max_workgroups);
+  c10::hip::HIPGuardMasqueradingAsCUDA guard(x.device().index());
+  auto y = at::empty({x.size(0), p.n, x.size(2), x.size(3)}, x.options(),
+                     at::MemoryFormat::ChannelsLast);
+  auto part = at::empty({p.splits, p.pstride}, x.options().dtype(at::kFloat));
+  launch_conv1x1_stats(p, x.data_ptr(), weight.data_ptr(), y.data_ptr(),
+                       part.data_ptr<float>(), bn_stream(x));
+  return {y, part};
+}
+
+py::dict py_conv1x1_plan(int64_t rows, int64_t k, int64_t n,
+                         int64_t max_workgroups) {
+  const Conv1x1Plan p = conv1x1_plan(rows, k, n, (int)max_workgroups);
+  py::dict d;
+  d["eligible"] = p.eligible;
+  d["native"] = p.native;
+  d["threads"] = kConvThreads;
+  d["tile_rows"] = kConvTileRows;
+  d["mfma_tiles"] = p.nt;
+  d["tile_channels"] = p.bn;
+  d["ntiles"] = p.ntiles;
+  d["k_chunk"] = p.kc;
+  d["k_chunks"] = p.nchunks;
+  d["resident"] = p.resident;
+  d["row_tiles"] = p.row_tiles;
+  d["splits"] = p.splits;
+  d["grid"] = p.grid;
+  d["tiles_per_split"] = p.tiles_per_split;
+  d["run"] = p.run;
+  d["lds_bytes"] = p.lds_bytes;
+  d["partial_stride"] = p.pstride;
+  d["partial_floats"] = p.partial_floats;
+  return d;
+}
+
+at::Tensor py_conv1x1_walk(int64_t rows, int64_t k, int64_t n,
+                           int64_t max_workgroups) {
+  const Conv1x1Plan p = conv1x1_plan(rows, k, n, (int)max_workgroups);
+  TORCH_CHECK(p.eligible, "conv1x1_walk: shape is not eligible");
+  auto out = at::full({p.grid, p.tiles_per_split, 4}, -1,
+                      at::TensorOptions().dtype(at::kLong));
+  int64_t* o = out.data_ptr<int64_t>();
+  for (int wg = 0; wg < p.grid; wg++) {
+    const int split = conv1x1_split(p, wg), nt = conv1x1_ntile(p, wg);
+    for (int i = 0; i < p.tiles_per_split; i++) {
+      const int t = conv1x1_tile(p, split, i);
+      if (t >= p.row_tiles) break;
+      int64_t* e = o + ((int64_t)wg * p.tiles_per_split + i) * 4;
+      e[0] = (int64_t)t * kConvTileRows;
+      e[1] = std::min<int64_t>(e[0] + kConvTileRows, p.rows);
+      e[2] = (int64_t)nt * p.bn;
+      e[3] = e[2] + p.bn;
+    }
+  }
+  return out;
 }
 
 void py_register_layer(int64_t bucket_idx, int64_t layer_idx, int64_t numel,
@@ -981,19 +1092,47 @@
   m.def("bn_act_forward", &cgx::py_bn_act_forward, py::arg("x"),
         py::arg("identity"), py::arg("weight"), py::arg("bias"),
         py::arg("running_mean"), py::arg("running_var"), py::arg("momentum"),
-        py::arg("eps"), py::arg("relu"),
+        py::arg("eps"), py::arg("relu"), py::arg("part") = py::none(),
         "Training-mode BatchNorm2d of a channels_last bf16 tensor, fused with "
         "an optional residual add and ReLU -> (out, mean, invstd, mask | "
-        "None); updates the running statistics in place.");
+        "None); updates the running statistics in place.  With `part`, the "
+        "partials conv1x1_stats returned with x, the statistics pass over x "
+        "is skipped.");
   m.def("bn_act_backward", &cgx::py_bn_act_backward, py::arg("dy"),
         py::arg("x"), py::arg("mean"), py::arg("invstd"), py::arg("weight"),
         py::arg("mask"), py::arg("has_identity"),
         "Backward of bn_act_forward -> (dx, dgamma, dbeta, didentity | None).");
-  m.def("bn_act2_forward", &cgx::py_bn_act2_forward,
+  m.def("bn_act2_forward", &cgx::py_bn_act2_forward, py::arg("x3"),
+        py::arg("xd"), py::arg("weight3"), py::arg("bias3"),
+        py::arg("running_mean3"), py::arg("running_var3"),
+        py::arg("momentum3"), py::arg("eps3"), py::arg("weightd"),
+        py::arg("biasd"), py::arg("running_meand"), py::arg("running_vard"),
+        py::arg("momentumd"), py::arg("epsd"), py::arg("relu"),
+        py::arg("part3") = py::none(), py::arg("partd") = py::none(),
         "relu(bn3(x3) + bn_d(xd)) with both BatchNorms in training mode: "
         "(x3, xd, weight3, bias3, running_mean3, running_var3, momentum3, "
         "eps3, weightd, biasd, running_meand, running_vard, momentumd, epsd, "
-        "relu) -> (out, mean3, invstd3, meand, invstdd, mask | None).");
+        "relu, part3=None, partd=None) -> (out, mean3, invstd3, meand, "
+        "invstdd, mask | None); part3 / partd as `part` of bn_act_forward.");
+  m.def("conv1x1_stats", &cgx::py_conv1x1_stats, py::arg("x"),
+        py::arg("weight"), py::arg("max_workgroups") = 0,
+        "conv2d(x, weight) of a 1x1 / stride 1 / no-bias convolution on a "
+        "channels_last bf16 tensor -> (y, part); part holds the per-channel "
+        "(count, mean, M2) partials of y.  max_workgroups > 0 caps the "
+        "persistent grid.");
+  m.def("conv1x1_eligible", &cgx::py_conv1x1_eligible, py::arg("x"),
+        py::arg("weight"),
+        "True where conv1x1_stats takes (x, weight): CUDA, bf16, dense "
+        "channels_last input, [N, K, 1, 1] weight, and a shape conv1x1_plan "
+        "calls eligible.");
+  m.def("conv1x1_plan", &cgx::py_conv1x1_plan, py::arg("rows"), py::arg("k"),
+        py::arg("n"), py::arg("max_workgroups") = 0,
+        "The launch geometry of conv1x1_stats for [rows, k] x [n, k], and "
+        "`native`: whether the model uses it at this shape.");
+  m.def("conv1x1_walk", &cgx::py_conv1x1_walk, py::arg("rows"), py::arg("k"),
+        py::arg("n"), py::arg("max_workgroups") = 0,
+        "Test seam: [grid, tiles_per_split, 4] int64, (row0, row1, n0, n1) "
+        "of every tile each workgroup visits (-1: none).");
   m.def("bn_act2_backward", &cgx::py_bn_act2_backward,
         "Backward of bn_act2_forward: (dy, x3, xd, mean3, invstd3, weight3, "
         "meand, invstdd, weightd, mask) -> (dx3, dxd, dgamma3, dbeta3, "
diff --git a/csrc/bn_kernels.hip b/csrc/bn_kernels.hip
--- a/csrc/bn_kernels.hip
+++ b/csrc/bn_kernels.hip
@@ -1,5 +1,6 @@
 #include <hip/hip_runtime.h>
 
+#include "bn_moments.h"
 #include "bn_plan.h"
 #include "check.h"
 
@@ -19,12 +20,6 @@
   f[7] = __uint_as_float(v.w & 0xffff0000u);
 }
 
-__device__ inline unsigned bf16_bits(float f) {
-  const unsigned u = __float_as_uint(f);
-  if ((u & 0x7fffffffu) > 0x7f800000u) return (u >> 16) | 0x40u;
-  return (u + 0x7fffu + ((u >> 16) & 1u)) >> 16;
-}
-
 __device__ inline uint4 pack8(const unsigned (&b)[8]) {
   return make_uint4(b[0] | (b[1] << 16), b[2] | (b[3] << 16),
                     b[4] | (b[5] << 16), b[6] | (b[7] << 16));
@@ -40,38 +35,6 @@
 #pragma unroll
   for (int j = 0; j < K; j++) dst[j] = src[j];
 }
-
-
-template <int K>
-struct Moments {
-  float n = 0.f;
-  float mean[K] = {};
-  float m2[K] = {};
-
-  __device__ void push(const float (&x)[K]) {
-    n += 1.f;
-    const float inv = __builtin_amdgcn_rcpf(n);
-#pragma unroll
-    for (int j = 0; j < K; j++) {
-      const float d = x[j] - mean[j];
-      mean[j] = fmaf(d, inv, mean[j]);
-      m2[j] = fmaf(d, x[j] - mean[j], m2[j]);
-    }
-  }
-
-  __device__ void merge(float nb, const float (&mb)[K], const float (&m2b)[K]) {
-    const float nt = n + nb;
-    const float fb = nt > 0.f ? nb / nt : 0.f;
-    const float w = n * fb;
-#pragma unroll
-    for (int j = 0; j < K; j++) {
-      const float d = mb[j] - mean[j];
-      mean[j] = fmaf(d, fb, mean[j]);
-      m2[j] = (m2[j] + m2b[j]) + (d * d) * w;
-    }
-    n = nt;
-  }
-};
 
 template <int K>
 __device__ inline void wg_merge(Moments<K>& m, float (*sh)[kT], int tid,
@@ -165,34 +128,33 @@
 constexpr int kFinLanes = kT / kBnFinChannels;
 
 __global__ __launch_bounds__(kT) void bn_stats_finalize(
-    const float* __restrict__ pmean, const float* __restrict__ pm2,
-    const float* __restrict__ pcnt, float* __restrict__ mean,
-    float* __restrict__ invstd, float* __restrict__ running_mean,
-    float* __restrict__ running_var, float momentum, float eps, BnPlan p) {
+    BnPartials q, float* __restrict__ mean, float* __restrict__ invstd,
+    float* __restrict__ running_mean, float* __restrict__ running_var,
+    float momentum, float eps) {
   __shared__ float sh[3][kT];
   const int tid = threadIdx.x;
   const int c = blockIdx.x * kBnFinChannels + tid % kBnFinChannels;
   const int lane = tid / kBnFinChannels;
   Moments<1> m;
-  if (c < p.channels) {
-    const int ct = (c / 8) / p.tc;
-    for (int s0 = lane; s0 < p.splits; s0 += 4 * kFinLanes) {
+  if (c < q.channels) {
+    const int ct = (c / 8) / q.tc;
+    for (int s0 = lane; s0 < q.splits; s0 += 4 * kFinLanes) {
       float nb[4], mb[4][1], m2b[4][1];
 #pragma unroll
       for (int u = 0; u < 4; u++) {
         const int s = s0 + u * kFinLanes;
-        const bool live = s < p.splits;
-        const int64_t o = (int64_t)s * p.channels + c;
-        nb[u] = live ? pcnt[s * p.ctiles + ct] : 0.f;
-        mb[u][0] = live ? pmean[o] : 0.f;
-        m2b[u][0] = live ? pm2[o] : 0.f;
+        const bool live = s < q.splits;
+        const int64_t o = (int64_t)s * q.pstride + c;
+        nb[u] = live ? q.cnt[(int64_t)s * q.cstride + ct] : 0.f;
+        mb[u][0] = live ? q.mean[o] : 0.f;
+        m2b[u][0] = live ? q.m2[o] : 0.f;
       }
 #pragma unroll
       for (int u = 0; u < 4; u++) m.merge(nb[u], mb[u], m2b[u]);
     }
   }
   wg_merge<1>(m, sh, tid, kBnFinChannels);
-  if (tid < kBnFinChannels && c < p.channels) {
+  if (tid < kBnFinChannels && c < q.channels) {
     const float var = m.m2[0] / m.n;
     mean[c] = m.mean[0];
     invstd[c] = 1.f / sqrtf(var + eps);
@@ -752,18 +714,30 @@
   return (p.channels + kBnFinChannels - 1) / kBnFinChannels;
 }
 
-void launch_bn_stats(const BnPlan& p, const void* x_, float* part, float* mean,
-                     float* invstd, float* running_mean, float* running_var,
-                     float momentum, float eps, hipStream_t stream) {
-  float* pmean = part;
-  float* pm2 = part + p.partial_floats;
-  float* pcnt = part + 2 * p.partial_floats;
-  const uint4* x = static_cast<const uint4*>(x_);
-  hipLaunchKernelGGL(bn_stats, dim3(p.grid), dim3(kT), 0, stream, x, pmean,
-                     pm2, pcnt, p);
+void launch_bn_stats(const BnPlan& p, const void* x_, float* part,
+                     const BnPartials* stats, float* mean, float* invstd,
+                     float* running_mean, float* running_var, float momentum,
+                     float eps, hipStream_t stream) {
+  BnPartials q;
+  if (stats) {
+    q = *stats;
+  } else {
+    float* pmean = part;
+    float* pm2 = part + p.partial_floats;
+    float* pcnt = part + 2 * p.partial_floats;
+    hipLaunchKernelGGL(bn_stats, dim3(p.grid), dim3(kT), 0, stream,
+                       static_cast<const uint4*>(x_), pmean, pm2, pcnt, p);
+    q.mean = pmean;
+    q.m2 = pm2;
+    q.cnt = pcnt;
+    q.channels = p.channels;
+    q.splits = p.splits;
+    q.tc = p.tc;
+    q.pstride = p.channels;
+    q.cstride = p.ctiles;
+  }
   hipLaunchKernelGGL(bn_stats_finalize, dim3(fin_grid(p)), dim3(kT), 0, stream,
-                     pmean, pm2, pcnt, mean, invstd, running_mean, running_var,
-                     momentum, eps, p);
+                     q, mean, invstd, running_mean, running_var, momentum, eps);
 }
 
 }
@@ -774,7 +748,7 @@
   const uint4* idn = static_cast<const uint4*>(a.identity);
   uint4* out = static_cast<uint4*>(a.out);
   const dim3 grid(p.grid), block(kT);
-  launch_bn_stats(p, a.x, a.part, a.mean, a.invstd, a.running_mean,
+  launch_bn_stats(p, a.x, a.part, a.stats, a.mean, a.invstd, a.running_mean,
                   a.running_var, a.momentum, a.eps, stream);
 #define CGX_BN_APPLY(RELU, ADD)                                              \
   hipLaunchKernelGGL((bn_apply<RELU, ADD>), grid, block, 0, stream, x, idn,  \
@@ -819,9 +793,9 @@
                             hipStream_t stream) {
   const BnOperand &a = j.a, &b = j.b;
   float* part_b = j.part + 2 * p.partial_floats + p.grid;
-  launch_bn_stats(p, a.x, j.part, a.mean, a.invstd, a.running_mean,
+  launch_bn_stats(p, a.x, j.part, a.stats, a.mean, a.invstd, a.running_mean,
                   a.running_var, a.momentum, a.eps, stream);
-  launch_bn_stats(p, b.x, part_b, b.mean, b.invstd, b.running_mean,
+  launch_bn_stats(p, b.x, part_b, b.stats, b.mean, b.invstd, b.running_mean,
                   b.running_var, b.momentum, b.eps, stream);
   const uint4* x3 = static_cast<const uint4*>(a.x);
   const uint4* xd = static_cast<const uint4*>(b.x);
@@ -875,7 +849,7 @@
 
 void launch_bn_pool_forward(const BnPlan& p, const BnPoolPlan& g,
                             const BnPoolArgs& a, hipStream_t stream) {
-  launch_bn_stats(p, a.x, a.part, a.mean, a.invstd, a.running_mean,
+  launch_bn_stats(p, a.x, a.part, nullptr, a.mean, a.invstd, a.running_mean,
                   a.running_var, a.momentum, a.eps, stream);
   hipLaunchKernelGGL(bn_apply_pool, dim3(g.grid), dim3(kT), 0, stream,
                      static_cast<const uint4*>(a.x), a.mean, a.invstd, a.weight,
diff --git a/csrc/bn_moments.h b/csrc/bn_moments.h
--- /dev/null
+++ b/csrc/bn_moments.h
@@ -0,0 +1,45 @@
+#pragma once
+
+#include <hip/hip_runtime.h>
+
+namespace cgx {
+
+__device__ inline unsigned bf16_bits(float f) {
+  const unsigned u = __float_as_uint(f);
+  if ((u & 0x7fffffffu) > 0x7f800000u) return (u >> 16) | 0x40u;
+  return (u + 0x7fffu + ((u >> 16) & 1u)) >> 16;
+}
+
+
+template <int K>
+struct Moments {
+  float n = 0.f;
+  float mean[K] = {};
+  float m2[K] = {};
+
+  __device__ void push(const float (&x)[K]) {
+    n += 1.f;
+    const float inv = __builtin_amdgcn_rcpf(n);
+#pragma unroll
+    for (int j = 0; j < K; j++) {
+      const float d = x[j] - mean[j];
+      mean[j] = fmaf(d, inv, mean[j]);
+      m2[j] = fmaf(d, x[j] - mean[j], m2[j]);
+    }
+  }
+
+  __device__ void merge(float nb, const float (&mb)[K], const float (&m2b)[K]) {
+    const float nt = n + nb;
+    const float fb = nt > 0.f ? nb / nt : 0.f;
+    const float w = n * fb;
+#pragma unroll
+    for (int j = 0; j < K; j++) {
+      const float d = mb[j] - mean[j];
+      mean[j] = fmaf(d, fb, mean[j]);
+      m2[j] = (m2[j] + m2b[j]) + (d * d) * w;
+    }
+    n = nt;
+  }
+};
+
+}
diff --git a/csrc/bn_plan.h b/csrc/bn_plan.h
--- a/csrc/bn_plan.h
+++ b/csrc/bn_plan.h
@@ -51,6 +51,17 @@
   return (int64_t)(wg / p.ctiles) * p.channels + (int64_t)cg * 8;
 }
 
+struct BnPartials {
+  const float* mean = nullptr;
+  const float* m2 = nullptr;
+  const float* cnt = nullptr;
+  int channels = 0;
+  int splits = 0;
+  int tc = 0;
+  int pstride = 0;
+  int cstride = 0;
+};
+
 struct BnForwardArgs {
   const void* x;
   const void* identity;
@@ -65,6 +76,7 @@
   float* invstd;
   uint8_t* mask;
   float* part;
+  const BnPartials* stats = nullptr;
 };
 void launch_bn_forward(const BnPlan& p, const BnForwardArgs& a,
                        hipStream_t stream);
@@ -97,6 +109,7 @@
   void* dx;
   float* dgamma;
   float* dbeta;
+  const BnPartials* stats = nullptr;
 };
 struct BnJoinArgs {
   BnOperand a, b;
diff --git a/csrc/conv1x1_kernels.hip b/csrc/conv1x1_kernels.hip
--- /dev/null
+++ b/csrc/conv1x1_kernels.hip
@@ -0,0 +1,225 @@
+#include <hip/hip_runtime.h>
+
+#include "bn_moments.h"
+#include "check.h"
+#include "conv1x1_plan.h"
+
+namespace cgx {
+namespace {
+
+constexpr int kT = kConvThreads;
+
+typedef __bf16 bf16x8 __attribute__((ext_vector_type(8)));
+typedef __bf16 bf16x2 __attribute__((ext_vector_type(2)));
+typedef float f32x2 __attribute__((ext_vector_type(2)));
+typedef float f32x16 __attribute__((ext_vector_type(16)));
+
+template <int KC>
+__device__ inline int w_slot(int n, int q) {
+  return n * (KC / 8) + (q ^ (KC == 64 ? (n >> 1) & 7 : n & 15));
+}
+
+__device__ inline int acc_row(int i, int h) {
+  return (i & 3) + 8 * (i >> 2) + 4 * h;
+}
+
+__device__ inline unsigned pack_bf16(float a, float b) {
+  const f32x2 f = {a, b};
+  return __builtin_bit_cast(unsigned, __builtin_convertvector(f, bf16x2));
+}
+
+template <int NT, int KC>
+__device__ inline void stage_w(uint4* dst, const uint4* __restrict__ w, int n0,
+                               int k, int chunk, int tid) {
+  constexpr int cpr = KC / 8;
+  for (int idx = tid; idx < 32 * NT * cpr; idx += kT) {
+    const int n = idx / cpr, q = idx % cpr;
+    dst[w_slot<KC>(n, q)] = w[((int64_t)(n0 + n) * k + chunk * KC) / 8 + q];
+  }
+}
+
+template <int NT, int KC, bool RES>
+__global__ __launch_bounds__(kT) void conv1x1_stats(
+    const uint4* __restrict__ x, const uint4* __restrict__ w,
+    uint4* __restrict__ y, float* __restrict__ part, Conv1x1Plan p) {
+  extern __shared__ uint4 lds[];
+  constexpr int BN = 32 * NT, cpr = KC / 8, steps = KC / 16;
+  constexpr int wchunks = BN * cpr;
+  const int tid = threadIdx.x, wave = tid >> 6, lane = tid & 63;
+  const int c = lane & 31, h = lane >> 5;
+  const int ntile = conv1x1_ntile(p, blockIdx.x);
+  const int split = conv1x1_split(p, blockIdx.x);
+  const int n0 = ntile * BN;
+  const int kvec = p.k / 8, nvec = p.n / 8;
+  uint4* stage = lds + (RES ? p.nchunks : 1) * wchunks + wave * 256;
+  unsigned* stage32 = reinterpret_cast<unsigned*>(stage);
+
+  if (RES) {
+    for (int kc = 0; kc < p.nchunks; kc++)
+      stage_w<NT, KC>(lds + kc * wchunks, w, n0, p.k, kc, tid);
+    __syncthreads();
+  }
+
+  auto a_row = [&](int t) {
+    int64_t r = (int64_t)t * kConvTileRows + wave * 32 + c;
+    r = r < p.rows ? r : p.rows - 1;
+    return x + r * kvec;
+  };
+
+  Moments<NT> st;
+  uint4 a[steps], an[steps];
+  const uint4* xr = a_row(split);
+#pragma unroll
+  for (int s = 0; s < steps; s++) a[s] = xr[2 * s + h];
+
+  for (int i = 0; i < p.tiles_per_split; i++) {
+    const int t = conv1x1_tile(p, split, i);
+    if (t >= p.row_tiles) break;
+    const int tn = conv1x1_tile(p, split, i + 1);
+    const uint4* xn = a_row(tn < p.row_tiles ? tn : t);
+
+    f32x16 acc[NT];
+#pragma unroll
+    for (int j = 0; j < NT; j++)
+#pragma unroll
+      for (int e = 0; e < 16; e++) acc[j][e] = 0.f;
+
+    for (int kc = 0; kc < p.nchunks; kc++) {
+      const uint4* src = kc + 1 < p.nchunks ? xr + (kc + 1) * cpr : xn;
+#pragma unroll
+      for (int s = 0; s < steps; s++) an[s] = src[2 * s + h];
+      if (!RES) {
+        __syncthreads();
+        stage_w<NT, KC>(lds, w, n0, p.k, kc, tid);
+        __syncthreads();
+      }
+      const uint4* wl = lds + (RES ? kc * wchunks : 0);
+#pragma unroll
+      for (int s = 0; s < steps; s++) {
+        const bf16x8 av = __builtin_bit_cast(bf16x8, a[s]);
+#pragma unroll
+        for (int j = 0; j < NT; j++) {
+          const uint4 b = wl[w_slot<KC>(j * 32 + c, 2 * s + h)];
+          acc[j] = __builtin_amdgcn_mfma_f32_32x32x16_bf16(
+              av, __builtin_bit_cast(bf16x8, b), acc[j], 0, 0, 0);
+        }
+      }
+#pragma unroll
+      for (int s = 0; s < steps; s++) a[s] = an[s];
+    }
+    xr = xn;
+
+    const int64_t r0 = (int64_t)t * kConvTileRows + wave * 32;
+    const int live = (int)(p.rows - r0 < 32 ? p.rows - r0 : 32);
+
+    unsigned pk[NT][8];
+#pragma unroll
+    for (int j = 0; j < NT; j++)
+#pragma unroll
+      for (int e = 0; e < 8; e++)
+        pk[j][e] = pack_bf16(acc[j][2 * e], acc[j][2 * e + 1]);
+
+#pragma unroll
+    for (int e = 0; e < 8; e++) {
+      float lo[NT], hi[NT];
+#pragma unroll
+      for (int j = 0; j < NT; j++) {
+        lo[j] = __uint_as_float(pk[j][e] << 16);
+        hi[j] = __uint_as_float(pk[j][e] & 0xffff0000u);
+      }
+      if (acc_row(2 * e, h) < live) st.push(lo);
+      if (acc_row(2 * e + 1, h) < live) st.push(hi);
+    }
+
+    const int odd = c & 1;
+#pragma unroll
+    for (int jp = 0; jp < NT / 2; jp++) {
+#pragma unroll
+      for (int jj = 0; jj < 2; jj++)
+#pragma unroll
+        for (int e = 0; e < 8; e++) {
+          const unsigned own = pk[2 * jp + jj][e];
+          const unsigned other = (unsigned)__builtin_amdgcn_update_dpp(
+              0, (int)own, 0xB1, 0xf, 0xf, false);
+          const unsigned word = odd ? (other >> 16) | (own & 0xffff0000u)
+                                    : (own & 0xffffu) | (other << 16);
+          const int row = acc_row(2 * e, h) + odd;
+          stage32[row * 32 + ((jj * 16 + (c >> 1)) ^ ((row & 1) << 4))] = word;
+        }
+      asm volatile("" ::: "memory");
+      __builtin_amdgcn_wave_barrier();
+#pragma unroll
+      for (int u = 0; u < 4; u++) {
+        const int idx = u * 64 + lane, row = idx >> 3, q = idx & 7;
+        const uint4 v = stage[row * 8 + (q ^ ((row & 1) << 2))];
+        if (row < live) y[(r0 + row) * nvec + (n0 + jp * 64) / 8 + q] = v;
+      }
+      asm volatile("" ::: "memory");
+      __builtin_amdgcn_wave_barrier();
+    }
+  }
+
+  __syncthreads();
+  float* sc = reinterpret_cast<float*>(lds);
+  const int run = wave * 2 + h;
+#pragma unroll
+  for (int j = 0; j < NT; j++) {
+    sc[run * BN + j * 32 + c] = st.mean[j];
+    sc[(8 + run) * BN + j * 32 + c] = st.m2[j];
+  }
+  if (c == 0) sc[16 * BN + run] = st.n;
+  __syncthreads();
+  if (tid < BN) {
+    Moments<1> m[8];
+#pragma unroll
+    for (int r = 0; r < 8; r++) {
+      m[r].n = sc[16 * BN + r];
+      m[r].mean[0] = sc[r * BN + tid];
+      m[r].m2[0] = sc[(8 + r) * BN + tid];
+    }
+#pragma unroll
+    for (int step = 1; step < 8; step *= 2)
+#pragma unroll
+      for (int r = 0; r < 8; r += 2 * step)
+        m[r].merge(m[r + step].n, m[r + step].mean, m[r + step].m2);
+    float* row = part + (int64_t)split * p.pstride;
+    row[n0 + tid] = m[0].mean[0];
+    row[p.n + n0 + tid] = m[0].m2[0];
+    if (tid == 0) row[2 * p.n + ntile] = m[0].n;
+  }
+}
+
+template <int NT, int KC, bool RES>
+void launch(const Conv1x1Plan& p, const void* x, const void* w, void* y,
+            float* part, hipStream_t stream) {
+  static const hipError_t attr = hipFuncSetAttribute(
+      reinterpret_cast<const void*>(&conv1x1_stats<NT, KC, RES>),
+      hipFuncAttributeMaxDynamicSharedMemorySize,
+      kConvWLdsBytes + kConvStageBytes);
+  CGX_HIP_CHECK(attr);
+  hipLaunchKernelGGL((conv1x1_stats<NT, KC, RES>), dim3(p.grid), dim3(kT),
+                     p.lds_bytes, stream, static_cast<const uint4*>(x),
+                     static_cast<const uint4*>(w), static_cast<uint4*>(y), part,
+                     p);
+}
+
+template <int NT>
+void launch_nt(const Conv1x1Plan& p, const void* x, const void* w, void* y,
+               float* part, hipStream_t stream) {
+  if (p.kc == 64) launch<NT, 64, true>(p, x, w, y, part, stream);
+  else if (p.resident) launch<NT, 128, true>(p, x, w, y, part, stream);
+  else launch<NT, 128, false>(p, x, w, y, part, stream);
+}
+
+}
+
+void launch_conv1x1_stats(const Conv1x1Plan& p, const void* x, const void* w,
+                          void* y, float* part, hipStream_t stream) {
+  TORCH_CHECK(p.eligible, "conv1x1_stats: shape is not eligible");
+  if (p.nt == 2) launch_nt<2>(p, x, w, y, part, stream);
+  else if (p.nt == 4) launch_nt<4>(p, x, w, y, part, stream);
+  else launch_nt<8>(p, x, w, y, part, stream);
+  CGX_HIP_CHECK(hipGetLastError());
+}
+
+}
diff --git a/csrc/conv1x1_plan.cc b/csrc/conv1x1_plan.cc
--- /dev/null
+++ b/csrc/conv1x1_plan.cc
@@ -0,0 +1,66 @@
+#include "conv1x1_plan.h"
+
+#include <algorithm>
+
+namespace cgx {
+namespace {
+
+struct Measured {
+  int k, n;
+  int64_t rows;
+};
+constexpr Measured kNative[] = {
+    {64, 64, 802816},   {64, 256, 802816},  {256, 64, 802816},
+    {256, 128, 802816}, {128, 512, 200704}, {512, 128, 200704},
+    {256, 1024, 50176},
+};
+
+bool measured_faster(int64_t rows, int k, int n) {
+  for (const Measured& m : kNative)
+    if (m.k == k && m.n == n && m.rows == rows) return true;
+  return false;
+}
+
+bool pow2_in(int64_t v, int64_t lo, int64_t hi) {
+  return v >= lo && v <= hi && (v & (v - 1)) == 0;
+}
+
+}
+
+Conv1x1Plan conv1x1_plan(int64_t rows, int64_t k, int64_t n,
+                         int max_workgroups) {
+  Conv1x1Plan p;
+  p.rows = rows;
+  p.eligible = pow2_in(k, 64, 2048) && pow2_in(n, 64, 2048) && rows >= 2 &&
+               rows <= kBnMaxRows;
+  if (!p.eligible) return p;
+  p.k = (int)k;
+  p.n = (int)n;
+  p.native = measured_faster(rows, p.k, p.n);
+
+  p.nt = std::min(p.n / 32, kConvMaxNt);
+  p.bn = 32 * p.nt;
+  p.ntiles = p.n / p.bn;
+  p.kc = p.k == 64 ? 64 : 128;
+  p.nchunks = p.k / p.kc;
+  p.resident = p.bn * p.k * 2 <= kConvWLdsBytes;
+  p.lds_bytes = p.bn * (p.resident ? p.k : p.kc) * 2 + kConvStageBytes;
+
+  p.row_tiles = (int)((rows + kConvTileRows - 1) / kConvTileRows);
+  const int by_regs = p.nt == 8 ? 1 : p.nt == 4 ? 2 : 3;
+  const int per_cu = std::max(1, std::min(kConvLdsBytes / p.lds_bytes, by_regs));
+  int64_t splits = std::min<int64_t>(
+      p.row_tiles, std::max(1, kConvCus * per_cu / p.ntiles));
+  splits = std::min(splits, std::max<int64_t>(1, rows / 82));
+  if (max_workgroups > 0)
+    splits = std::min<int64_t>(splits, std::max(1, max_workgroups / p.ntiles));
+  p.splits = (int)splits;
+  p.grid = p.ntiles * p.splits;
+  p.tiles_per_split = (p.row_tiles + p.splits - 1) / p.splits;
+  p.run = 16 * p.tiles_per_split;
+  p.pstride = 2 * p.n + p.ntiles;
+  p.partial_floats = (int64_t)p.splits * p.pstride;
+  return p;
+}
+
+}
diff --git a/csrc/conv1x1_plan.h b/csrc/conv1x1_plan.h
--- /dev/null
+++ b/csrc/conv1x1_plan.h
@@ -0,0 +1,68 @@
+#pragma once
+
+#include <cstdint>
+
+#include "bn_plan.h"
+
+namespace cgx {
+
+constexpr int kConvThreads = 256;
+constexpr int kConvTileRows = 128;
+constexpr int kConvMaxNt = 8;
+constexpr int kConvCus = 256;
+constexpr int kConvLdsBytes = 160 * 1024;
+constexpr int kConvWLdsBytes = 128 * 1024;
+constexpr int kConvStageBytes = 16 * 1024;
+
+struct Conv1x1Plan {
+  int64_t rows = 0;
+  int k = 0, n = 0;
+  bool eligible = false;
+  bool native = false;
+  int nt = 0;
+  int bn = 0;
+  int ntiles = 0;
+  int kc = 0;
+  int nchunks = 0;
+  bool resident = false;
+  int row_tiles = 0;
+  int splits = 0;
+  int grid = 0;
+  int tiles_per_split = 0;
+  int run = 0;
+  int lds_bytes = 0;
+  int pstride = 0;
+  int64_t partial_floats = 0;
+};
+
+Conv1x1Plan conv1x1_plan(int64_t rows, int64_t k, int64_t n,
+                         int max_workgroups = 0);
+
+__host__ __device__ inline int conv1x1_ntile(const Conv1x1Plan& p, int wg) {
+  return wg % p.ntiles;
+}
+__host__ __device__ inline int conv1x1_split(const Conv1x1Plan& p, int wg) {
+  return wg / p.ntiles;
+}
+__host__ __device__ inline int conv1x1_tile(const Conv1x1Plan& p, int split,
+                                            int i) {
+  return split + i * p.splits;
+}
+
+inline BnPartials conv1x1_partials(const float* part, int n, int splits,
+                                   int ntiles) {
+  BnPartials q;
+  q.mean = part;
+  q.m2 = part + n;
+  q.cnt = part + 2 * n;
+  q.channels = n;
+  q.splits = splits;
+  q.tc = n / ntiles / 8;
+  q.pstride = q.cstride = 2 * n + ntiles;
+  return q;
+}
+
+void launch_conv1x1_stats(const Conv1x1Plan& p, const void* x, const void* w,
+                          void* y, float* part, hipStream_t stream);
+
+}
diff --git a/torch_cgx_amd/models/resnet.py b/torch_cgx_amd/models/resnet.py
--- a/torch_cgx_amd/models/resnet.py
+++ b/torch_cgx_amd/models/resnet.py
@@ -4,7 +4,7 @@
 import torch
 import torch.nn as nn
 
-from ..ops.fused_bn import bn_act, bn_act_pool
+from ..ops.fused_bn import bn_act, bn_act_pool, conv_bn_act
 
 
 class Bottleneck(nn.Module):
@@ -26,13 +26,13 @@
 
     def forward(self, x):
         identity = x
-        out = bn_act(self.bn1, self.conv1(x))
+        out = conv_bn_act(self.conv1, self.bn1, x)
         out = bn_act(self.bn2, self.conv2(out))
-        out = self.conv3(out)
         if self.downsample is not None:
             conv, bn = self.downsample[0], self.downsample[1]
-            return bn_act(self.bn3, out, conv(x), identity_bn=bn)
-        return bn_act(self.bn3, out, identity)
+            return conv_bn_act(self.conv3, self.bn3, out, identity,
+                               identity_conv=conv, identity_bn=bn)
+        return conv_bn_act(self.conv3, self.bn3, out, identity)
 
 
 class ResNet(nn.Module):
diff --git a/torch_cgx_amd/ops/fused_bn.py b/torch_cgx_amd/ops/fused_bn.py
--- a/torch_cgx_amd/ops/fused_bn.py
+++ b/torch_cgx_amd/ops/fused_bn.py
@@ -12,10 +12,10 @@
 class _BnAct(torch.autograd.Function):
     @staticmethod
     def forward(ctx, x, identity, weight, bias, running_mean, running_var,
-                momentum, eps, relu):
+                momentum, eps, relu, part):
         out, mean, invstd, mask = _C.bn_act_forward(
             x, identity, weight, bias, running_mean, running_var, momentum,
-            eps, relu)
+            eps, relu, part)
         ctx.save_for_backward(x, mean, invstd, weight, mask)
         ctx.has_identity = identity is not None
         return out
@@ -25,17 +25,19 @@
         x, mean, invstd, weight, mask = ctx.saved_tensors
         dx, dgamma, dbeta, didentity = _C.bn_act_backward(
             dy, x, mean, invstd, weight, mask, ctx.has_identity)
-        return (dx, didentity, dgamma, dbeta, None, None, None, None, None)
+        return (dx, didentity, dgamma, dbeta, None, None, None, None, None,
+                None)
 
 
 class _BnActJoin(torch.autograd.Function):
     @staticmethod
     def forward(ctx, x, xd, weight, bias, running_mean, running_var, momentum,
                 eps, weightd, biasd, running_meand, running_vard, momentumd,
-                epsd, relu):
+                epsd, relu, part, partd):
         out, mean, invstd, meand, invstdd, mask = _C.bn_act2_forward(
             x, xd, weight, bias, running_mean, running_var, momentum, eps,
-            weightd, biasd, running_meand, running_vard, momentumd, epsd, relu)
+            weightd, biasd, running_meand, running_vard, momentumd, epsd, relu,
+            part, partd)
         ctx.save_for_backward(x, xd, mean, invstd, weight, meand, invstdd,
                               weightd, mask)
         return out
@@ -47,7 +49,7 @@
         dx, dxd, dgamma, dbeta, dgammad, dbetad = _C.bn_act2_backward(
             dy, x, xd, mean, invstd, weight, meand, invstdd, weightd, mask)
         return (dx, dxd, dgamma, dbeta, None, None, None, None, dgammad,
-                dbetad, None, None, None, None, None)
+                dbetad, None, None, None, None, None, None, None)
 
 
 class _BnActPool(torch.autograd.Function):
@@ -93,18 +95,21 @@
 
 def bn_act(bn: torch.nn.BatchNorm2d, x: torch.Tensor,
            identity: torch.Tensor = None, relu: bool = True,
-           identity_bn: torch.nn.BatchNorm2d = None) -> torch.Tensor:
+           identity_bn: torch.nn.BatchNorm2d = None,
+           part: torch.Tensor = None,
+           identity_part: torch.Tensor = None) -> torch.Tensor:
     if identity_bn is not None:
         if _native(bn, x, identity) and _native(identity_bn, identity, x):
             bn.num_batches_tracked.add_(1)
             identity_bn.num_batches_tracked.add_(1)
             return _BnActJoin.apply(x, identity, *_bn_args(bn),
-                                    *_bn_args(identity_bn), relu)
+                                    *_bn_args(identity_bn), relu, part,
+                                    identity_part)
         out = bn(x) + identity_bn(identity)
         return F.relu(out, inplace=True) if relu else out
     if _native(bn, x, identity):
         bn.num_batches_tracked.add_(1)
-        return _BnAct.apply(x, identity, *_bn_args(bn), relu)
+        return _BnAct.apply(x, identity, *_bn_args(bn), relu, part)
     out = bn(x)
     if identity is not None:
         out = out + identity
@@ -113,6 +118,79 @@
     return out
 
 
+class _Conv1x1Stats(torch.autograd.Function):
+
+    @staticmethod
+    @torch.amp.custom_fwd(device_type="cuda", cast_inputs=torch.bfloat16)
+    def forward(ctx, x, weight):
+        y, part = _C.conv1x1_stats(x, weight)
+        ctx.save_for_backward(x, weight)
+        ctx.mark_non_differentiable(part)
+        return y, part
+
+    @staticmethod
+    @torch.amp.custom_bwd(device_type="cuda")
+    def backward(ctx, dy, _dpart):
+        x, weight = ctx.saved_tensors
+        dx, dw, _ = torch.ops.aten.convolution_backward(
+            dy, x, weight, None, (1, 1), (0, 0), (1, 1), False, (0, 0), 1,
+            (ctx.needs_input_grad[0], ctx.needs_input_grad[1], False))
+        return dx, dw
+
+
+def native_conv1x1_mode() -> str:
+    if not fused_bn_enabled():
+        return "0"
+    return os.environ.get("CGX_NATIVE_CONV1X1", "1")
+
+
+def _conv1x1_native(conv, bn, x) -> bool:
+    mode = native_conv1x1_mode()
+    if mode == "0":
+        return False
+    if not (type(conv) is torch.nn.Conv2d and conv.kernel_size == (1, 1)
+            and conv.stride == (1, 1) and conv.padding == (0, 0)
+            and conv.dilation == (1, 1) and conv.groups == 1
+            and conv.bias is None and conv.padding_mode == "zeros"):
+        return False
+    if not (bn.training and bn.track_running_stats
+            and bn.momentum is not None and bn.weight is not None
+            and bn.bias is not None and bn.weight.dtype == torch.float32):
+        return False
+    if not (x.is_cuda and x.dim() == 4 and x.dtype == torch.bfloat16
+            and _C.bn_eligible(x)):
+        return False
+    w = conv.weight
+    autocast = (torch.is_autocast_enabled("cuda")
+                and torch.get_autocast_dtype("cuda") == torch.bfloat16)
+    if not (w.device == x.device and w.shape[1] == x.shape[1]
+            and (w.dtype == torch.bfloat16
+                 or (autocast and w.dtype == torch.float32))):
+        return False
+    if w.dtype == torch.bfloat16 and not _C.conv1x1_eligible(x, w):
+        return False
+    plan = _C.conv1x1_plan(x.numel() // x.shape[1], x.shape[1], w.shape[0])
+    return plan["eligible"] and (plan["native"] or mode == "all")
+
+
+def _conv(conv, bn, x):
+    if _conv1x1_native(conv, bn, x):
+        return _Conv1x1Stats.apply(x, conv.weight)
+    return conv(x), None
+
+
+def conv_bn_act(conv: torch.nn.Conv2d, bn: torch.nn.BatchNorm2d,
+                x: torch.Tensor, identity: torch.Tensor = None,
+                relu: bool = True, identity_conv: torch.nn.Conv2d = None,
+                identity_bn: torch.nn.BatchNorm2d = None) -> torch.Tensor:
+    y, part = _conv(conv, bn, x)
+    if identity_conv is None:
+        return bn_act(bn, y, identity, relu, part=part)
+    yd, partd = _conv(identity_conv, identity_bn, identity)
+    return bn_act(bn, y, yd, relu, identity_bn=identity_bn, part=part,
+                  identity_part=partd)
+
+
 def _pool_is_3x3_s2_p1(pool) -> bool:
     def pair(v):
         return tuple(v) if isinstance(v, (tuple, list)) else (v, v)
```

Measured after the change: 7751 samples/s (median of 6 runs). 3.4% higher.
